# Roy-Kid/ADMP

Measured on AMD Instinct MI355X. Metric: ns/day (electrostatics get_forces per 1 fs step, polarizable PME incl. SCF, moving atoms), higher is better.
Workload: dtype f64; 1 GPU; water_pol_1024 (BASELINE configs[1]): 1024 polarizable MPID waters = 3072 atoms, seeded liquid box L=31.289 A, rc 4 A, f64; n_atoms=3072, n_pairs=42510, pair_list=fixed during the timed steps, parallelism=single GPU

## Files before the change

### admp_amd/_lib.py

```python
import ctypes

import numpy as np
import os

_HERE = os.path.dirname(os.path.abspath(__file__))
LIB_PATH = os.environ.get('ADMP_HIP_LIB') or os.path.join(_HERE, 'lib', 'libadmp_hip.so')

_c = ctypes
_vp, _i32, _i64, _dbl = _c.c_void_p, _c.c_int, _c.c_int64, _c.c_double
_u32, _u64 = _c.c_uint32, _c.c_uint64
_dp = _c.POINTER(_c.c_double)
_ip = _c.POINTER(_c.c_int)

PROTOTYPES = {
    'admp_version': (_c.c_char_p, []),
    'admp_create': (_i32, [_c.POINTER(_vp), _i32, _i32]),
    'admp_destroy': (_i32, [_vp]),
    'admp_last_error': (_c.c_char_p, [_vp]),
    'admp_set_stream': (_i32, [_vp, _vp]),
    'admp_use_default_stream': (_i32, [_vp]),
    'admp_synchronize': (_i32, [_vp]),
    'admp_set_topology': (_i32, [_vp, _i32, _vp, _vp, _vp, _vp, _vp]),
    'admp_set_ewald': (_i32, [_vp, _dbl, _i32, _i32, _i32, _i32, _i32]),
    'admp_set_pairs': (_i32, [_vp, _i64, _vp, _i32]),
    'admp_share_neighbors': (_i32, [_vp, _vp]),
    'admp_num_pairs': (_i64, [_vp]),
    'admp_set_cutoff': (_i32, [_vp, _dbl]),
    'admp_set_dipole_source': (_i32, [_vp, _vp]),
    'admp_pme_energy_grad': (_i32, [_vp, _vp, _dp, _vp, _vp, _vp, _i32, _dp, _dp, _dp, _vp, _i32, _dbl, _dp, _vp, _vp,
                                    _ip, _ip, _i32]),
    'admp_pme_energy_fixed_dipoles': (_i32, [_vp, _vp, _dp, _vp, _vp, _vp, _i32, _dp, _dp, _vp, _dp, _vp, _vp, _vp]),
    'admp_pme_box_grad': (_i32, [_vp, _vp, _dp, _vp, _vp, _vp, _i32, _dp, _dp, _vp, _dp, _dp]),
    'admp_disp_box_grad': (_i32, [_vp, _vp, _dp, _vp, _i32, _i32, _dp, _dp, _dp]),
    'admp_tt_box_grad': (_i32, [_vp, _vp, _dp, _vp, _i32, _dp, _dp, _dp]),
    'admp_local_frames': (_i32, [_vp, _vp, _dp, _vp]),
    'admp_set_option': (_i32, [_vp, _i32, _i32]),
    'admp_disp_energy_grad': (_i32, [_vp, _vp, _dp, _vp, _i32, _i32, _dp, _dp, _vp, _i32]),
    'admp_prune_pairs': (_i32, [_vp, _vp, _dp, _dbl]),
    'admp_disp_set_types': (_i32, [_vp, _i32, _vp, _dp]),
    'admp_tt_energy_grad': (_i32, [_vp, _vp, _dp, _vp, _i32, _dp, _dp, _vp, _i32]),
    'admp_pair_program_build': (_i32, [_vp, _c.c_char_p, _i32, _ip]),
    'admp_pair_program_energy_grad': (_i32, [_vp, _i32, _vp, _dp, _vp, _i32, _dp, _dp, _vp, _i32]),
    'admp_disp_param_grad': (_i32, [_vp, _vp, _dp, _vp, _i32, _i32, _dp, _vp]),
    'admp_tt_param_grad': (_i32, [_vp, _vp, _dp, _vp, _i32, _dp, _vp]),
    'admp_thole_sums': (_i32, [_vp, _vp, _dp, _vp, _vp, _vp, _i32, _dp, _dp, _vp, _vp, _vp]),
    'admp_pscale_grad': (_i32, [_vp, _vp, _dp, _vp, _vp, _vp, _i32, _dp, _dp, _vp, _dp]),
    'admp_mscale_grad': (_i32, [_vp, _i32, _vp, _dp, _vp, _i32, _i32, _dp, _i32]),
    'admp_md_bonded': (_i32, [_vp, _vp, _dp, _i32, _vp, _vp, _i32, _vp, _vp, _vp, _vp]),
    'admp_md_kick_drift': (_i32, [_vp, _i32, _vp, _vp, _vp, _vp, _dbl, _dbl, _vp]),
    'admp_md_langevin': (_i32, [_vp, _i32, _vp, _vp, _vp, _vp, _dbl, _dbl, _dbl, _dbl, _u64, _u64, _vp]),
    'admp_md_random': (_i32, [_vp, _i32, _i64, _u64, _u64, _u32, _vp]),
    'admp_md_bonded_box': (_i32, [_vp, _vp, _dp, _i32, _vp, _vp, _i32, _vp, _vp, _vp, _vp]),
    'admp_md_virial': (_i32, [_vp, _i32, _vp, _vp, _vp, _vp, _u64, _u64, _vp]),
    'admp_md_scale': (_i32, [_vp, _i32, _vp, _vp, _dbl]),
    'admp_md_mts_plan': (_i32, [_vp, _i32, _i32, _vp, _vp, _i32, _vp, _vp, _i32]),
    'admp_md_mts_step': (_i32, [_vp, _i32, _vp, _vp, _vp, _vp, _dp, _dbl, _dbl, _i32, _dbl, _dbl, _u64, _u64, _vp, _vp]),
    'admp_md_mts_info': (_i32, [_vp, _c.POINTER(_i64)]),
    'admp_md_con_plan': (_i32, [_vp, _i32, _i32, _vp, _vp, _i32]),
    'admp_md_con_step': (_i32, [_vp, _i32, _vp, _vp, _vp, _vp, _dp, _dbl, _dbl, _dbl, _dbl, _u64, _u64, _dbl, _i32, _vp]),
    'admp_md_con_kick': (_i32, [_vp, _i32, _vp, _vp, _vp, _vp, _dp, _dbl, _dbl, _dbl, _i32, _vp, _vp]),
    'admp_md_con_project': (_i32, [_vp, _i32, _vp, _vp, _vp, _dp, _dbl, _i32, _vp]),
    'admp_md_con_info': (_i32, [_vp, _c.POINTER(_i64)]),
    'admp_md_mol_plan': (_i32, [_vp, _i32, _vp, _i32]),
    'admp_md_mol_sums': (_i32, [_vp, _i32, _vp, _vp, _vp, _vp, _dp, _u64, _u64, _vp]),
    'admp_md_mol_scale': (_i32, [_vp, _i32, _vp, _vp, _vp, _dp, _dbl, _dbl]),
    'admp_md_mol_info': (_i32, [_vp, _c.POINTER(_i64)]),
    'admp_md_fire_step': (_i32, [_vp, _i32, _vp, _vp, _vp, _vp, _dp, _dbl, _u64, _vp]),
    'admp_md_vrescale': (_i32, [_vp, _i32, _vp, _vp, _vp, _dbl, _i64, _dbl, _dbl, _u64, _u64, _u64, _vp]),
    'admp_neighbor_count': (_i32, [_vp, _i32, _vp, _dp, _dbl, _c.POINTER(_i64)]),
    'admp_neighbor_fill': (_i32, [_vp, _vp]),
    'admp_set_pairs_from_positions': (_i32, [_vp, _vp, _dp, _dbl]),
    'admp_slab_configure': (_i32, [_vp, _i32, _i32]),
    'admp_slab_info': (_i32, [_vp, _c.POINTER(_i64)]),
    'admp_scf_stats': (_i32, [_vp, _c.POINTER(_i64), _i32]),
    'admp_scf_aspc': (_i32, [_vp, _i32, _i32, _dbl]),
    'admp_scf_aspc_reset': (_i32, [_vp]),
    'admp_scf_aspc_info': (_i32, [_vp, _c.POINTER(_i64), _dp]),
    'admp_xpass_stats':(_i32, [_vp, _c.POINTER(_i64), _i32]),
    'admp_plane_mfma_stats': (_i32, [_vp, _c.POINTER(_i64), _i32]),
    'admp_plane_mfma_stats4': (_i32, [_vp, _c.POINTER(_i64), _i32]),
    'admp_mesh_convolve': (_i32, [_vp, _dp, _i32, _vp, _i32, _dp, _ip]),
    'admp_slab_mesh_convolve': (_i32, [_vp, _dp, _i32, _vp, _i32, _dp, _ip]),
    'admp_slab_lists': (_i32, [_vp, _i32, _i32, _ip, _ip, _ip, _ip, _ip, _ip, _ip, _ip, _ip, _c.POINTER(_i64)]),
    'admp_pair_real': (_i32, [_vp, _vp, _dp, _vp, _vp, _vp, _i32, _dp, _dp, _vp, _vp, _i32, _i32, _i32, _dp, _vp, _vp, _vp, _ip]),
    'admp_pair_rider_stats': (_i32, [_vp, _c.POINTER(_i64), _i32]),
    'admp_mesh_spread': (_i32, [_vp, _vp, _dp, _vp, _vp, _vp, _vp, _i32, _i32, _i32, _vp, _ip]),
    'admp_mesh_gather': (_i32, [_vp, _vp, _dp, _vp, _vp, _vp, _vp, _vp, _i32, _i32, _dp, _vp, _vp, _vp, _ip]),
    'admp_set_comm': (_i32, [_vp, _vp]),
    'admp_slab_home': (_i32, [_vp, _vp, _ip, _ip]),
    'admp_rccl_unique_id': (_i32, [_vp]),
    'admp_rccl_create': (_i32, [_c.POINTER(_vp), _i32, _vp, _i32, _i32]),
    'admp_rccl_destroy': (_i32, [_vp]),
    'admp_rccl_abort': (_i32, [_vp]),
    'admp_rccl_stats': (_i32, [_vp, _c.POINTER(_i64), _c.POINTER(_i64), _i32]),
    'admp_rccl_all_reduce': (_i32, [_vp, _vp, _i64, _i32, _i32, _vp]),
    'admp_rccl_all_to_all_v': (_i32, [_vp, _vp, _c.POINTER(_i64), _vp, _c.POINTER(_i64), _i32, _vp]),
    'admp_rccl_shift': (_i32, [_vp, _vp, _vp, _i64, _i32, _i32, _vp]),
    'admp_rccl_version': (_i32, [_ip]),
    'admp_rccl_last_error': (_c.c_char_p, []),
    'admp_set_comm_rccl': (_i32, [_vp, _vp]),
    'admp_profile_enable': (_i32, [_vp, _i32]),
    'admp_profile_filter': (_i32, [_vp, _c.c_char_p]),
    'admp_profile_reset': (_i32, [_vp]),
    'admp_profile_count': (_i32, [_vp]),
    'admp_profile_entry': (_i32, [_vp, _i32, _c.POINTER(_c.c_char_p), _dp, _c.POINTER(_i64)]),
}

T_I32, T_F32, T_F64 = 0, 1, 2
OP_SUM, OP_MAX = 0, 1
TAGS = {1: 'ghost_planes', 2: 'transpose', 3: 'halo_dipoles', 4: 'halo_gradient', 5: 'scf_max', 6: 'energies',
        7: 'replicate_outputs'}
_i64p = _c.POINTER(_i64)
ALL_REDUCE_FN = _c.CFUNCTYPE(_i32, _vp, _vp, _i64, _i32, _i32, _i32)
ALL_TO_ALL_V_FN = _c.CFUNCTYPE(_i32, _vp, _vp, _i64p, _vp, _i64p, _i32, _i32)
SHIFT_FN = _c.CFUNCTYPE(_i32, _vp, _vp, _vp, _i64, _i32, _i32, _i32)


class AdmpComm(_c.Structure):
    _fields_ = [('ctx', _vp), ('all_reduce', ALL_REDUCE_FN), ('all_to_all_v', ALL_TO_ALL_V_FN), ('shift', SHIFT_FN)]


OPT_REFERENCE_KPOINTS = 1
OPT_KEEP_POL_SITES = 2
OPT_SIDE_STREAM = 3
OPT_ASPC_HOLD = 4
E_ARG, E_STATE = -1, -5
RCCL_ID_BYTES, RCCL_NTAGS = 128, 8
MESH_INFO_WORDS = 16
MESH_PATHS = ('rocfft', 'fused_x', 'direct_lines', 'direct_planes', 'two_level')

SPREAD_FORMS = ('scan', 'planes', 'bricks', 'plane_kernel')

_lib = None


class AdmpHipError(RuntimeError):
    pass


def load():
    global _lib
    if _lib is not None:
        return _lib
    if not os.path.exists(LIB_PATH):
        raise ImportError(
            'admp_amd: %s not found. Build it with `python -m admp_amd.build` (needs hipcc); '
            'there is no CPU fallback for the PME path.' % LIB_PATH)
    lib = ctypes.CDLL(LIB_PATH)
    for name, (res, args) in PROTOTYPES.items():
        fn = getattr(lib, name)
        fn.restype = res
        fn.argtypes = args
    _lib = lib
    return lib


def check(handle, rc, what):
    if rc != 0:
        msg = load().admp_last_error(handle)
        raise AdmpHipError('%s failed (code %d): %s' % (what, rc, msg.decode() if msg else ''))


def darr(values):
# ... 3 lines not shown
```

### admp_amd/csrc/atom_kernels.hip

```cpp
#include <cstdlib>

#include <cstring>

#include "launch.h"
#include "reduce.h"

namespace admp {

constexpr int kAtomBlock = 256;

template <class T>
__device__ __forceinline__ void load3(const T* a, int i, T o[3]) {
  o[0] = a[3 * i]; o[1] = a[3 * i + 1]; o[2] = a[3 * i + 2];
}

template <class T>
__device__ __forceinline__ void frame_of(const Topology& top, const T* pos, const Box<T>& box, int i, int& type,
                                         int& iz, int& ix, int& iy, FrameWork<T>& w) {
  type = top.axis_type[i];
  iz = top.axis_idx[3 * i];
  ix = top.axis_idx[3 * i + 1];
  iy = top.axis_idx[3 * i + 2];
  T p[3], pz[3] = {0, 0, 0}, px[3] = {0, 0, 0}, py[3] = {0, 0, 0};
  load3(pos, i, p);
  if (iz >= 0) load3(pos, iz, pz); else if (type != NoAxisType) type = NoAxisType;
  if (ix >= 0) load3(pos, ix, px);
  if (iy >= 0) load3(pos, iy, py);
  local_frame_fwd(type, box, p, pz, px, py, w);
}

template <class T>
__global__ __launch_bounds__(kAtomBlock) void k_prepare_sites(Topology top, const T* __restrict__ pos,
                                                              const T* __restrict__ Qlocal,
                                                              const T* __restrict__ Ucart, const T* __restrict__ pol,
                                                              const T* __restrict__ thole, Box<T> box,
                                                              Site<T>* __restrict__ sites, double* zero_next,
                                                              RecipGeom<T> g, int4* __restrict__ bases,
                                                              int* __restrict__ act_list, int* __restrict__ act_count,
                                                              const int* __restrict__ cls, int* __restrict__ cls_flags,
                                                              RQ4<T>* __restrict__ rq, T* __restrict__ Ucopy,
                                                              const int* __restrict__ list, int nlist) {
  int i = blockIdx.x * kAtomBlock + threadIdx.x;
  if (zero_next && i < E_WORDS) zero_next[i] = 0.0;
  if (list) {
    if (i >= nlist) return;
    i = list[i];
  }
  if (act_list) {
    __shared__ int wcnt[kAtomBlock / 64], wbase;
    const bool act = i < top.na && pol && pol[i] > T(0);
    const unsigned long long m = __ballot(act);
    const int lane = threadIdx.x & 63, wave = threadIdx.x >> 6;
    if (lane == 0) wcnt[wave] = __popcll(m);
    __syncthreads();
    if (threadIdx.x == 0) {
      int tot = 0;
      for (int w = 0; w < kAtomBlock / 64; ++w) { const int c = wcnt[w]; wcnt[w] = tot; tot += c; }
      wbase = tot ? atomicAdd(act_count, tot) : 0;
    }
    __syncthreads();
    if (act) act_list[wbase + wcnt[wave] + __popcll(m & ((1ull << lane) - 1ull))] = i;
  }
  if (i >= top.na) return;
  int type, iz, ix, iy;
  FrameWork<T> w;
  frame_of(top, pos, box, i, type, iz, ix, iy, w);
  T ql[9], cx[3], cy[3], cz[3];
#pragma unroll
  for (int k = 0; k < 9; ++k) ql[k] = Qlocal[9 * i + k];
  Site<T> s;
  frame_cols(w.X, w.Y, w.Z, cx, cy, cz);
  rot_harm(ql, cx, cy, cz, s.Q);
  load3(pos, i, s.r);
  if (Ucart) {
    s.U[0] = Ucart[3 * i + 2]; s.U[1] = Ucart[3 * i]; s.U[2] = Ucart[3 * i + 1];
    if (Ucopy) { Ucopy[3 * i] = s.U[1]; Ucopy[3 * i + 1] = s.U[2]; Ucopy[3 * i + 2] = s.U[0]; }
  } else {
    s.U[0] = s.U[1] = s.U[2] = T(0);
  }
  T a = pol ? pol[i] : T(0);
  s.p6 = a > T(0) ? (T)pow((double)a, 1.0 / 6.0) : T(0);
  s.thole = thole ? thole[i] : T(0);
  s.pad[0] = s.pad[1] = s.pad[2] = T(0);
  if (s.p6 == T(0) && s.U[0] == T(0) && s.U[1] == T(0) && s.U[2] == T(0)) {
    bool mono = true;
#pragma unroll
    for (int k = 1; k < 9; ++k) mono = mono && ql[k] == T(0);
    s.pad[0] = mono ? T(1) : T(0);
  }
  if (cls_flags) {
    const bool was = cls && cls[i] != 0, is = s.pad[0] == T(1) && s.p6 == T(0);
    const int f = was && !is ? CLS_STALE : (!was && is ? CLS_BETTER : 0);
    if (f && !(*(volatile int*)cls_flags & f)) atomicOr(cls_flags, f);
  }
  sites[i] = s;
  if (rq) { RQ4<T> q; q.v[0] = s.r[0]; q.v[1] = s.r[1]; q.v[2] = s.r[2]; q.v[3] = s.Q[0]; rq[i] = q; }
  if (bases) {
    int b[3];
#pragma unroll
    for (int d = 0; d < 3; ++d) grid_ref(g, s.r, d, b[d]);
    const int dims[3] = {g.nloc0, g.K[1], g.K[2]};
    bases[i] = make_int4(b[0], b[1], b[2], brick_code(b, dims, make_bricks(dims)));
  }
}

template <class T>
__global__ __launch_bounds__(kAtomBlock) void k_site_classes(int na, const Site<T>* __restrict__ sites, int* __restrict__ cls) {
  const int i = blockIdx.x * kAtomBlock + threadIdx.x;
  if (i < na) cls[i] = site_is_mono(sites[i]) ? 1 : 0;
}

template <class T>
__global__ __launch_bounds__(kAtomBlock) void k_jacobi_delta(int n_act, const int* __restrict__ act,
                                                             const T* __restrict__ pol, const T* __restrict__ field,
                                                             T* __restrict__ Ucart, Site<T>* __restrict__ sites,
                                                             Site<T>* __restrict__ isites,
                                                             const unsigned long long* __restrict__ gate,
                                                             unsigned long long gate_bits, T relax) {
  const int slot = blockIdx.x * kAtomBlock + threadIdx.x;
  if (slot >= n_act) return;
  const int i = act[slot];
  const bool on = !gate || *gate >= gate_bits;
  const T s = on ? -pol[i] * T(1.0 / kDielectric) * relax : T(0);
  const T dx = field[3 * i] * s, dy = field[3 * i + 1] * s, dz = field[3 * i + 2] * s;
  Ucart[3 * i] += dx; Ucart[3 * i + 1] += dy; Ucart[3 * i + 2] += dz;
  Site<T> r = sites[i];
  r.U[0] += dz; r.U[1] += dx; r.U[2] += dy;
  r.pad[0] = dz; r.pad[1] = dx; r.pad[2] = dy;
  sites[i] = r;
#pragma unroll
  for (int k = 0; k < 9; ++k) r.Q[k] = T(0);
  r.U[0] = dz; r.U[1] = dx; r.U[2] = dy;
  isites[slot] = r;
}

template <class T>
__global__ __launch_bounds__(kAtomBlock) void k_aspc_predict(long n, AspcSets<T> h, T* __restrict__ out) {
  const long i = (long)blockIdx.x * kAtomBlock + threadIdx.x;
  if (i >= n) return;
  double acc = 0.0;
#pragma unroll
  for (int j = 0; j < kAspcMaxSets; ++j)
    if (j < h.n) acc += h.B[j] * (double)h.U[j][i];
  out[i] = (T)acc;
}

template <class T>
__global__ __launch_bounds__(kAtomBlock) void k_local_frames(Topology top, const T* __restrict__ pos, Box<T> box,
                                                             T* __restrict__ out) {
  int i = blockIdx.x * kAtomBlock + threadIdx.x;
  if (i >= top.na) return;
  int type, iz, ix, iy;
  FrameWork<T> w;
  frame_of(top, pos, box, i, type, iz, ix, iy, w);
#pragma unroll
  for (int k = 0; k < 3; ++k) { out[9 * i + k] = w.X[k]; out[9 * i + 3 + k] = w.Y[k]; out[9 * i + 6 + k] = w.Z[k]; }
}
template <class T>
void launch_local_frames(hipStream_t st, const Topology& top, const T* pos, const Box<T>& box, T* out) {
  k_local_frames<T><<<(top.na + kAtomBlock - 1) / kAtomBlock, kAtomBlock, 0, st>>>(top, pos, box, out);
}
template void launch_local_frames<float>(hipStream_t, const Topology&, const float*, const Box<float>&, float*);
template void launch_local_frames<double>(hipStream_t, const Topology&, const double*, const Box<double>&, double*);

template <class T>
__global__ __launch_bounds__(kAtomBlock) void k_field_finish(int na, const Site<T>* __restrict__ sites,
                                                             const T* __restrict__ pol, const T* __restrict__ Ucart,
                                                             const T* __restrict__ fld_pair,
                                                             const T* __restrict__ fld_recip, T kappa,
                                                             T* __restrict__ field, unsigned long long* fmax_bits,
                                                             const int* __restrict__ list, const int* __restrict__ n_dev) {
  const int slot = blockIdx.x * kAtomBlock + threadIdx.x;
  if (n_dev) na = min(na, *n_dev);
  double fm = 0.0;
  if (slot < na) {
    const int i = list ? list[slot] : slot;
    const T a = pol[i];
    T fx, fy, fz;
    total_field(sites[i], a, Ucart + 3 * i, fld_pair + 3 * i, fld_recip + 3 * i, kappa, fx, fy, fz);
    field[3 * i] = fx; field[3 * i + 1] = fy; field[3 * i + 2] = fz;
    if (a > T(0.001)) fm = fmax(fabs((double)fx), fmax(fabs((double)fy), fabs((double)fz)));
  }
  fm = block_reduce_max<kAtomBlock>(fm);
  if (threadIdx.x == 0 && fm > 0.0) atomicMax(fmax_bits, nonneg_bits(fm));
}

template <class T>
__global__ __launch_bounds__(kAtomBlock) void k_finish(Topology top, const T* __restrict__ pos, Box<T> box,
                                                       const Site<T>* __restrict__ sites, const T* __restrict__ pol,
                                                       const T* __restrict__ Ucart, int lpol, T kappa,
                                                       T* __restrict__ pot, T* __restrict__ grad,
                                                       T* __restrict__ dQlocal, double* energies,
                                                       const int* __restrict__ list, int nlist) {
  const int slot = blockIdx.x * kAtomBlock + threadIdx.x;
  double eself = 0.0, epen = 0.0;
  if (slot < nlist) {
    const int i = list ? list[slot] : slot;
    T f[3];
    self_factors(kappa, f);
    const Site<T>& s = sites[i];
    T Qt[9], P[9];
#pragma unroll
    for (int k = 0; k < 9; ++k) { Qt[k] = s.Q[k]; P[k] = pot[9 * i + k]; }
    if (lpol) { Qt[1] += s.U[0]; Qt[2] += s.U[1]; Qt[3] += s.U[2]; }
// ... 371 lines not shown
    FrameWork<T> w;
    frame_of(top, pos, box, i, type, iz, ix, iy, w);
    if (type != NoAxisType) {
      T f[3], P[9], tau[3], gp[3], gz[3], gx[3], gy[3], p[3];
      self_factors(kappa, f);
      total_potential(sites[i], pot + 9 * (size_t)i, lpol, f, P, nullptr);
      multipole_torque(P, sites[i].Q, tau);
      local_frame_bwd(type, w, tau, gp, gz, gx, gy);
      load3(pos, i, p);
      const int member[3] = {iz, type != Zonly ? ix : -1, (type == ZBisect || type == ThreeFold) ? iy : -1};
      const T* gk[3] = {gz, gx, gy};
      for (int m = 0; m < 3; ++m) {
        if (member[m] < 0) continue;
        T q[3], sh[3];
        load3(pos, member[m], q);
        const T d[3] = {q[0] - p[0], q[1] - p[1], q[2] - p[2]};
        if (!image_shift(box, d, sh)) continue;
        for (int a = 0; a < 3; ++a)
          for (int b = 0; b < 3; ++b) acc[3 * a + b] += (double)sh[a] * (double)gk[m][b];
      }
    }
  }
#pragma unroll
  for (int k = 0; k < 9; ++k) {
    const double v = block_reduce_sum<kAtomBlock>(acc[k]);
    if (threadIdx.x == 0 && v != 0.0) atomicAdd(&vir[k], v);
  }
}

template <class T>
__global__ __launch_bounds__(kAtomBlock) void k_scalar_sites(int na, const T* __restrict__ pos, const T* __restrict__ vals,
                                                             int stride, int chan, SelfCoefs self_coefs,
                                                             Site<T>* __restrict__ sites, double* energies, RecipGeom<T> g,
                                                             int4* __restrict__ bases) {
  chan += blockIdx.y;
  sites += (size_t)blockIdx.y * na;
  const double self_coef = self_coefs.c[blockIdx.y];
  const int i = blockIdx.x * kAtomBlock + threadIdx.x;
  double s2 = 0.0;
  if (i < na) {
    Site<T> s;
    load3(pos, i, s.r);
    const T c = vals[(long)stride * i + chan];
    s.Q[0] = c;
#pragma unroll
    for (int k = 1; k < 9; ++k) s.Q[k] = T(0);
    s.U[0] = s.U[1] = s.U[2] = T(0);
    s.p6 = s.thole = T(0);
    s.pad[0] = s.pad[1] = s.pad[2] = T(0);
    sites[i] = s;
    s2 = (double)c * (double)c;
    if (bases && blockIdx.y == 0) {
      int b[3];
#pragma unroll
      for (int d = 0; d < 3; ++d) grid_ref(g, s.r, d, b[d]);
      const int dims[3] = {g.nloc0, g.K[1], g.K[2]};
      bases[i] = make_int4(b[0], b[1], b[2], brick_code(b, dims, make_bricks(dims)));
    }
  }
  s2 = block_reduce_sum<kAtomBlock>(s2);
  if (threadIdx.x == 0) atomicAdd(&energies[E_SELF], self_coef * s2);
}

template <class T>
__global__ __launch_bounds__(kAtomBlock) void k_scale_add(int na, const T* __restrict__ vals, int stride, int chan,
                                                          const T* __restrict__ v, T* __restrict__ grad, int nch) {
  const int i = blockIdx.x * kAtomBlock + threadIdx.x;
  if (i >= na) return;
  T gx = 0, gy = 0, gz = 0;
  for (int b = 0; b < nch; ++b) {
    const T c = vals[(long)stride * i + chan + b];
    const T* vb = v + (size_t)b * 3 * na;
    gx += c * vb[3 * i]; gy += c * vb[3 * i + 1]; gz += c * vb[3 * i + 2];
  }
  grad[3 * i] += gx; grad[3 * i + 1] += gy; grad[3 * i + 2] += gz;
}

static inline int nblk(int n) { return (n + kAtomBlock - 1) / kAtomBlock; }

template <class T>
void launch_prepare_sites(hipStream_t st, const Topology& top, const T* pos, const T* Qlocal, const T* Ucart,
                          const T* pol, const T* thole, const Box<T>& box, Site<T>* sites, double* zero_next,
                          const RecipGeom<T>& g, int4* bases, int* act_list, int* act_count, const int* cls,
                          int* cls_flags, RQ4<T>* rq, T* Ucopy, const int* list, int nlist) {
  const int n = list ? nlist : top.na;
  if (n <= 0 && !zero_next) return;
  k_prepare_sites<T><<<nblk(n > E_WORDS || !zero_next ? (n > 0 ? n : 1) : E_WORDS), kAtomBlock, 0, st>>>(
      top, pos, Qlocal, Ucart, pol, thole, box, sites, zero_next, g, bases, list ? nullptr : act_list,
      list ? nullptr : act_count, cls, cls_flags, rq, Ucopy, list, nlist);
}
template <class T>
void launch_site_classes(hipStream_t st, int na, const Site<T>* sites, int* cls) {
  if (na > 0) k_site_classes<T><<<nblk(na), kAtomBlock, 0, st>>>(na, sites, cls);
}
template <class T>
void launch_field_finish(hipStream_t st, int na, const Site<T>* sites, const T* pol, const T* Ucart, const T* fld_pair,
                         const T* fld_recip, T kappa, T* field, unsigned long long* fmax_bits, const int* list,
                         const int* n_dev) {
  k_field_finish<T><<<nblk(na), kAtomBlock, 0, st>>>(na, sites, pol, Ucart, fld_pair, fld_recip, kappa, field, fmax_bits, list,
                                                     n_dev);
}
template <class T>
void launch_jacobi_delta(hipStream_t st, int n_act, const int* act, const T* pol, const T* field, T* Ucart, Site<T>* sites,
                         Site<T>* isites, const unsigned long long* gate, double gate_min, double relax) {
  unsigned long long bits;
  std::memcpy(&bits, &gate_min, sizeof(bits));
  if (n_act > 0)
    k_jacobi_delta<T><<<nblk(n_act), kAtomBlock, 0, st>>>(n_act, act, pol, field, Ucart, sites, isites, gate, bits, (T)relax);
}
template <class T>
void launch_aspc_predict(hipStream_t st, long n, const AspcSets<T>& h, T* out) {
  if (n > 0) k_aspc_predict<T><<<(unsigned)((n + kAtomBlock - 1) / kAtomBlock), kAtomBlock, 0, st>>>(n, h, out);
}
template <class T>
void launch_finish(hipStream_t st, const Topology& top, const T* pos, const Box<T>& box, const Site<T>* sites,
                   const T* pol, const T* Ucart, int lpol, T kappa, T* pot, T* grad, T* dQlocal, double* energies,
                   const int* list, int nlist, const FieldFin<T>& ff, const int* slab_bits) {
  const int gmin = env_int("ADMP_FINISH_GROUPS_MIN", 8192);
  if ((!list || slab_bits) && top.ngroups > 0 && top.na > gmin) {
    if (top.rows_blk && env_flag("ADMP_FINISH_ROWS", true))
      k_finish_rows<T><<<top.nrowblk < 1024 ? top.nrowblk : 1024, kFinishBlock, 0, st>>>(top, box, sites, pol, lpol, kappa, pot, grad,
                                                                                         dQlocal, energies, ff,
                                                                                         list ? slab_bits : nullptr);
    else
      k_finish_groups<T><<<nblk(top.ngroups), kAtomBlock, 0, st>>>(top, pos, box, sites, pol, Ucart, lpol, kappa, pot, grad,
                                                                   dQlocal, energies, ff, list ? slab_bits : nullptr);
    return;
  }
  if (!list && top.inv_ptr)
  {
    static const int lanes4_max = env_int("ADMP_FINISH4_MAX", 8192);
    if (top.na <= lanes4_max)
      k_finish_pull<T, 4><<<nblk(4 * top.na), kAtomBlock, 0, st>>>(top, pos, box, sites, pol, Ucart, lpol, kappa, pot, grad,
                                                                   dQlocal, energies, ff);
    else
      k_finish_pull<T, 1><<<nblk(top.na), kAtomBlock, 0, st>>>(top, pos, box, sites, pol, Ucart, lpol, kappa, pot, grad,
                                                               dQlocal, energies, ff);
  }
  else
    k_finish<T><<<nblk(nlist), kAtomBlock, 0, st>>>(top, pos, box, sites, pol, Ucart, lpol, kappa, pot, grad, dQlocal,
                                                    energies, list, nlist);
}

template <class T>
void launch_frame_virial(hipStream_t st, const Topology& top, const T* pos, const Box<T>& box, const Site<T>* sites,
                         int lpol, T kappa, const T* pot, double* vir, const int* list, int nlist) {
  const int n = list ? nlist : top.na;
  if (n > 0) k_frame_virial<T><<<nblk(n), kAtomBlock, 0, st>>>(top, pos, box, sites, lpol, kappa, pot, vir, list, nlist);
}
template void launch_frame_virial<float>(hipStream_t, const Topology&, const float*, const Box<float>&, const Site<float>*,
                                         int, float, const float*, double*, const int*, int);
template void launch_frame_virial<double>(hipStream_t, const Topology&, const double*, const Box<double>&,
                                          const Site<double>*, int, double, const double*, double*, const int*, int);

template <class T>
void launch_scalar_sites(hipStream_t st, int na, const T* pos, const T* vals, int stride, int chan, double self_coef,
                         Site<T>* sites, double* energies) {
  SelfCoefs sc;
  sc.c[0] = self_coef;
  k_scalar_sites<T><<<nblk(na), kAtomBlock, 0, st>>>(na, pos, vals, stride, chan, sc, sites, energies, RecipGeom<T>(), nullptr);
}
template <class T>
void launch_scalar_sites_batch(hipStream_t st, int na, const T* pos, const T* vals, int stride, int nch,
                               const double* self_coefs, Site<T>* sites, double* energies, const RecipGeom<T>* g, int4* bases) {
  SelfCoefs sc;
  for (int b = 0; b < nch && b < 3; ++b) sc.c[b] = self_coefs[b];
  k_scalar_sites<T><<<dim3(nblk(na), nch), kAtomBlock, 0, st>>>(na, pos, vals, stride, 0, sc, sites, energies,
                                                                 g ? *g : RecipGeom<T>(), g ? bases : nullptr);
}
template <class T>
void launch_scale_add(hipStream_t st, int na, const T* vals, int stride, int chan, const T* v, T* grad, int nch) {
  k_scale_add<T><<<nblk(na), kAtomBlock, 0, st>>>(na, vals, stride, chan, v, grad, nch);
}

#define INST(T)                                                                                                        \
  template void launch_scalar_sites<T>(hipStream_t, int, const T*, const T*, int, int, double, Site<T>*, double*);      \
  template void launch_scale_add<T>(hipStream_t, int, const T*, int, int, const T*, T*, int);                           \
  template void launch_scalar_sites_batch<T>(hipStream_t, int, const T*, const T*, int, int, const double*, Site<T>*,   \
                                             double*, const RecipGeom<T>*, int4*);                                      \
  template void launch_prepare_sites<T>(hipStream_t, const Topology&, const T*, const T*, const T*, const T*, const T*, \
                                        const Box<T>&, Site<T>*, double*, const RecipGeom<T>&, int4*, int*, int*,       \
                                        const int*, int*, RQ4<T>*, T*, const int*, int);                                \
  template void launch_site_classes<T>(hipStream_t, int, const Site<T>*, int*);                                         \
  template void launch_field_finish<T>(hipStream_t, int, const Site<T>*, const T*, const T*, const T*, const T*, T, T*,  \
                                       unsigned long long*, const int*, const int*);                                    \
  template void launch_jacobi_delta<T>(hipStream_t, int, const int*, const T*, const T*, T*, Site<T>*, Site<T>*,        \
                                       const unsigned long long*, double, double);                                    \
  template void launch_aspc_predict<T>(hipStream_t, long, const AspcSets<T>&, T*);                                      \
  template void launch_finish<T>(hipStream_t, const Topology&, const T*, const Box<T>&, const Site<T>*, const T*,        \
                                 const T*, int, T, T*, T*, T*, double*, const int*, int, const FieldFin<T>&, const int*);
INST(float)
INST(double)
#undef INST

}
```

### admp_amd/csrc/dft_kernels.hip

```cpp
#include "dft_lines.h"
#include "env.h"
#include "mfma.h"
#include "plane_mfma_plan.h"

namespace admp {

int dft_tile_cols(int N) { return dft_cols(N, dft_kq(), 0, 0); }
template <class T, int KQ, int JS>
__global__ __launch_bounds__(kDftBlock) void k_dft_z_r2c(int N, int nlines, int NL, int TK, const T* __restrict__ mesh,
                                                        Cx<T>* __restrict__ spec, const Cx<T>* __restrict__ twg,
                                                        long mesh_stride, long spec_stride) {
  mesh += blockIdx.y * mesh_stride;
  spec += blockIdx.y * spec_stride;
  const int H = (N - 1) / 2, Kh = N / 2 + 1;
  Cx<T>* tw = reinterpret_cast<Cx<T>*>(dft_smem);
  Cx<T>* p = tw + N;
  T* x0 = reinterpret_cast<T*>(p + H * NL);
  T* xn = x0 + NL;
  const int line0 = blockIdx.x * NL;
  const int nl = min(NL, nlines - line0);
  for (int t = threadIdx.x; t < N; t += kDftBlock) tw[t] = twg[t];
  for (int t = threadIdx.x; t < H * nl; t += kDftBlock) {
    const int l = t / H, jj = t - l * H;
    const T* x = mesh + (long)(line0 + l) * N;
// ... 225 lines not shown
  __syncthreads();
  double e = 0.0;
  auto combine = [&](Cx<T>* s, const T* G) {
    Cx<T> y[NTP];
#pragma unroll
    for (int ty = 0; ty < NTP; ++ty) y[ty] = Cx<T>{T(0), T(0)};
    double en = 0.0;
#pragma unroll
    for (int ch = 0; ch < 3; ++ch) {
      if (ch >= mix.nch) break;
      Cx<T> Sp{T(0), T(0)};
#pragma unroll
      for (int ty = 0; ty < NTP; ++ty) { const T cc = (T)mix.c[ch][ty]; Sp.re += cc * s[ty].re; Sp.im += cc * s[ty].im; }
      en += (double)G[ch] * ((double)Sp.re * Sp.re + (double)Sp.im * Sp.im);
#pragma unroll
      for (int ty = 0; ty < NTP; ++ty) { const T cg = (T)mix.c[ch][ty] * G[ch]; y[ty].re += cg * Sp.re; y[ty].im += cg * Sp.im; }
    }
#pragma unroll
    for (int ty = 0; ty < NTP; ++ty) s[ty] = y[ty];
    return en;
  };
#pragma unroll
  for (int u = 0; u < KQ; ++u) {
    const int t = threadIdx.x + u * kDftBlock;
    if (t >= H * NCt) continue;
    const int jj = t / NCt, cc = t - jj * NCt;
    Cx<T> s1[NTP], s2[NTP];
#pragma unroll
    for (int ty = 0; ty < NTP; ++ty) s1[ty] = s2[ty] = Cx<T>{T(0), T(0)};
    if (cc < ncp) {
      const int k1 = 1 + jj, k2 = N - 1 - jj, kz = col0 + cc;
#pragma unroll
      for (int ty = 0; ty < NTP; ++ty) { s1[ty] = S[k1 * NC + ty * NCt + cc]; s2[ty] = S[k2 * NC + ty * NCt + cc]; }
      const double w = (kz == 0 || ((K3 & 1) == 0 && kz == K3 / 2)) ? 0.5 : 1.0;
      const T G1[3] = {Gp[u][0][0], Gp[u][1][0], Gp[u][2][0]}, G2[3] = {Gp[u][0][1], Gp[u][1][1], Gp[u][2][1]};
      e += w * (combine(s1, G1) + combine(s2, G2));
    }
#pragma unroll
    for (int ty = 0; ty < NTP; ++ty)
      ab[jj * NC + ty * NCt + cc] = PairCx<T>{s1[ty].re + s2[ty].re, s1[ty].im + s2[ty].im, s1[ty].re - s2[ty].re, s1[ty].im - s2[ty].im};
  }
  if ((int)threadIdx.x < NCt) {
    const int cc = threadIdx.x;
    Cx<T> a[NTP], b[NTP];
#pragma unroll
    for (int ty = 0; ty < NTP; ++ty) a[ty] = b[ty] = Cx<T>{T(0), T(0)};
    if (cc < ncp) {
      const int kz = col0 + cc;
      const double w = (kz == 0 || ((K3 & 1) == 0 && kz == K3 / 2)) ? 0.5 : 1.0;
#pragma unroll
      for (int ty = 0; ty < NTP; ++ty) a[ty] = S[ty * NCt + cc];
      e += w * combine(a, G0);
      if ((N & 1) == 0) {
#pragma unroll
        for (int ty = 0; ty < NTP; ++ty) b[ty] = S[(N / 2) * NC + ty * NCt + cc];
        e += w * combine(b, Gn);
      }
    }
#pragma unroll
    for (int ty = 0; ty < NTP; ++ty) { x0[ty * NCt + cc] = a[ty]; xn[ty * NCt + cc] = b[ty]; }
  }
  __syncthreads();
  if (task) {
    Cx<T> Xk[KQ], Xnk[KQ];
    dft_pair_outputs_js<T, +1, KQ, JS>(N, k, NC, ab + c, x0[c], xn[c], tw, half, Xk, Xnk);
    Cx<T>* sp = spec + (long)cty * spec_tstride + base + ccol;
#pragma unroll
    for (int q = 0; q < KQ; ++q) {
      const int kq = g + q * TK;
      if (kq < Kh) {
        if (JS == 1 || half == 0) sp[(long)kq * jstride] = Xk[q];
        if ((JS == 1 || half == 1) && kq != 0 && 2 * kq != N) sp[(long)(N - kq) * jstride] = Xnk[q];
      }
    }
  }
  e = block_reduce_sum<kDftBlock>(e);
  if (threadIdx.x == 0) atomicAdd(&energies[slot], e);
}

constexpr int kZyBlock = 1024;

#ifdef ADMP_ZY_TRACE
__device__ long long* g_zy_trace;
#define ZY_TRACE(slot) do { if (threadIdx.x == 0) g_zy_trace[((blockIdx.z * gridDim.y + blockIdx.y) * gridDim.x + blockIdx.x) * 8 + (slot)] = wall_clock64(); } while (0)
#define ZY_TRACE_END(slot) do { __syncthreads(); ZY_TRACE(slot); } while (0)
#else
#define ZY_TRACE(slot) do {} while (0)
#define ZY_TRACE_END(slot) do {} while (0)
#endif

template <class T>
struct ZyLayout {
  size_t tw3, tw2, a, x0, b, total;
  __host__ __device__ ZyLayout(int N2, int N3) {
    const size_t H3 = (size_t)(N3 - 1) / 2, Kh = (size_t)N3 / 2 + 1;
    tw3 = 0;
    tw2 = tw3 + sizeof(Cx<T>) * N3;
    a = tw2 + sizeof(Cx<T>) * N2;
    const size_t fa = sizeof(Cx<T>) * H3 * N2, ia = sizeof(Cx<T>) * N2 * Kh;
    x0 = a + (fa > ia ? fa : ia);
    b = x0 + sizeof(Cx<T>) * N2;
    total = b + sizeof(Cx<T>) * N2 * Kh;
  }
};

constexpr int kZyW = 42;
constexpr int kZyScan = 3;
constexpr int kZySpreadMaxAtoms = 8192;
template <class T>
__host__ __device__ inline int zy_spread_sub(int N2, int N3) {
  const int Kh = N3 / 2 + 1;
  const long spare = (long)sizeof(Cx<T>) * N2 * Kh - (long)sizeof(unsigned short) * kZyScan * kZyBlock;
  const long n = spare / (long)(kZyW * sizeof(T) + 2 * sizeof(int));
  return n > kZyBlock / 3 ? kZyBlock / 3 : (int)n;
}
template <class T>
__device__ __forceinline__ void zy_plane_spread(const PlaneSpread<T>& sp, int px, int N2, int N3, Cx<T>* p, T* x0, T* xn,
                                                unsigned char* scratch, int SUB) {
  __shared__ int s_nhit;
  unsigned short* hits = reinterpret_cast<unsigned short*>(scratch);
  T* wts = reinterpret_cast<T*>(hits + kZyScan * kZyBlock);
  int* ebase = reinterpret_cast<int*>(wts + (size_t)SUB * kZyW);
  const int H3 = (N3 - 1) / 2;
  const Site<T>* sites = sp.sites + (size_t)blockIdx.y * sp.na;
  for (int t = threadIdx.x; t < H3 * N2; t += kZyBlock) p[t] = Cx<T>{T(0), T(0)};
  for (int t = threadIdx.x; t < 2 * N2; t += kZyBlock) x0[t] = T(0);
  const RecipGeom<T>& g = sp.g;
  for (int c0 = 0; c0 < sp.na; c0 += kZyScan * kZyBlock) {
    if (threadIdx.x == 0) s_nhit = 0;
    __syncthreads();
    int bx[kZyScan];
#pragma unroll
    for (int r = 0; r < kZyScan; ++r) {
      const int i = c0 + (int)threadIdx.x + r * kZyBlock;
      bx[r] = -1000;
      if (i < sp.na) {
        if (sp.bases) bx[r] = sp.bases[i].x;
        else {
          const T rr[3] = {sites[i].r[0], sites[i].r[1], sites[i].r[2]};
          (void)grid_ref(g, rr, 0, bx[r]);
        }
      }
    }
#pragma unroll
    for (int r = 0; r < kZyScan; ++r) {
      int a = px - bx[r];
      if (a < 0) a += g.K[0];
      if (bx[r] >= 0 && a < 6)
        hits[atomicAdd(&s_nhit, 1)] = (unsigned short)((c0 + (int)threadIdx.x + r * kZyBlock) | (a << 13));
    }
    __syncthreads();
    const int nhit = s_nhit;
    const int nsub = (nhit + SUB - 1) / SUB, per = nsub > 0 ? (nhit + nsub - 1) / nsub : 0;
    for (int sub = 0; sub < nhit; sub += per) {
      const int cnt = min(per, nhit - sub);
      if ((int)threadIdx.x < 3 * cnt) {
        const int e = threadIdx.x / 3, part = threadIdx.x - 3 * e;
        const int h = hits[sub + e];
        const Site<T>& site = sites[h & 0x1fff];
        T* w = wts + e * kZyW;
        const T r[3] = {site.r[0], site.r[1], site.r[2]};
        int base;
        T M[6], D1[6], D2[6], D3[6];
        const T f = grid_ref(g, r, part, base);
        bspline6(f, M, D1, D2, D3);
        if (part == 0) {
          const int a = h >> 13;
          T m0 = T(0), d0 = T(0), e0 = T(0);
#pragma unroll
          for (int k = 0; k < 6; ++k)
            if (k == a) { m0 = M[k]; d0 = D1[k]; e0 = D2[k]; }
          T Q[9], c1[3], c2[6];
#pragma unroll
          for (int k = 0; k < 9; ++k) Q[k] = site.Q[k];
          if (sp.lpol) { Q[1] += site.U[0]; Q[2] += site.U[1]; Q[3] += site.U[2]; }
          fold_multipole(g, Q, c1, c2);
          w[0] = Q[0] * m0 + c1[0] * d0 + c2[0] * e0;
          w[1] = c1[1] * m0 + c2[3] * d0;
          w[2] = c2[1] * m0;
          w[3] = c1[2] * m0 + c2[4] * d0;
          w[4] = c2[5] * m0;
          w[5] = c2[2] * m0;
        } else {
          const int o = part == 1 ? 6 : 24;
#pragma unroll
          for (int k = 0; k < 6; ++k) { w[o + k] = M[k]; w[o + 6 + k] = D1[k]; w[o + 12 + k] = D2[k]; }
          ebase[2 * e + part - 1] = base;
        }
      }
      __syncthreads();
      for (int task = threadIdx.x; task < cnt * 6; task += kZyBlock) {
        const int e = task / 6, b = task - e * 6;
        const T* w = wts + e * kZyW;
        const T m1 = w[6 + b], d1 = w[12 + b], e1 = w[18 + b];
        const T P0 = w[0] * m1 + w[1] * d1 + w[2] * e1;
        const T P1 = w[3] * m1 + w[4] * d1;
        const T P2 = w[5] * m1;
        const int jb = wrap_add(ebase[2 * e], b, N2), bz = ebase[2 * e + 1];
#pragma unroll
        for (int c = 0; c < 6; ++c) {
          const T v = P0 * w[24 + c] + P1 * w[30 + c] + P2 * w[36 + c];
          const int jc = wrap_add(bz, c, N3);
          T* dst;
          if (jc == 0) dst = &x0[jb];
          else if (jc <= H3) dst = &p[(jc - 1) * N2 + jb].re;
          else if (2 * jc == N3) dst = &xn[jb];
          else dst = &p[(N3 - 1 - jc) * N2 + jb].im;
          atomicAdd(dst, v);
        }
      }
      __syncthreads();
    }
  }
  for (int t = threadIdx.x; t < H3 * N2; t += kZyBlock) {
    const Cx<T> ab = p[t];
    p[t] = Cx<T>{ab.re + ab.im, ab.re - ab.im};
  }
}

template <class T, int SIGN>
__device__ __forceinline__ void dft_y_unit_rows(int N, int H, int KP, int ncols, int ib, int kl, int ct, bool w0, bool wn,
                                                const Cx<T>* Z, const Cx<T>* tw, Cx<T>* out, int os) {
  typedef typename Mfma<T>::Acc Acc;
  const int lane = threadIdx.x & 63, hi = plane_mfma_pos0(lane);
  const int i = ib + (lane & 15), c = plane_mfma_col(ct, lane), comp = plane_mfma_comp(lane);
  TwIdx ti(i < kl ? i : 0, hi, N);
  const bool live = c < ncols;
  const T* zc = reinterpret_cast<const T*>(Z + (live ? c : 0)) + comp;
  const int rs = 2 * ncols;
  struct Ops { Cx<T> w; T b[2]; };
  auto fetch = [&](Ops& o, int kk) {
    o.w = tw[ti.m];
    ti.step();
    const bool ok = live && kk < H;
    o.b[0] = ok ? zc[(1 + kk) * rs] : T(0);
    o.b[1] = ok ? zc[(N - 1 - kk) * rs] : T(0);
  };
  Acc P = {0, 0, 0, 0}, R = {0, 0, 0, 0};
  T s0 = T(0);
  auto mul = [&](const Ops& o) {
    s0 += o.b[0];
    P = Mfma<T>::mma(o.w.re, o.b[0], P);
    R = Mfma<T>::mma(o.w.im, o.b[1], R);
  };
  Ops A, B;
  fetch(A, hi);
  for (int kk = hi; kk < KP; kk += 8) {
    const bool two = kk + 4 < KP;
    if (two) fetch(B, kk + 4);
    mul(A);
    if (kk + 8 < KP) fetch(A, kk + 8);
    if (two) mul(B);
  }
  const T x0 = zc[0], xn = (N & 1) ? T(0) : zc[(N / 2) * rs];
  T* o = reinterpret_cast<T*>(out + (live ? c : 0)) + comp;
#pragma unroll
  for (int r = 0; r < 4; ++r) {
    const int k = 1 + ib + (lane >> 4) + 4 * r;
    const T other = __shfl_xor(R[r], 8, 64);
    if (live && k <= kl) {
      T base = x0 + P[r];
      if ((N & 1) == 0) base += (k & 1) ? -xn : xn;
      const T q = comp ? T(SIGN) * other : -T(SIGN) * other;
      o[2 * (long)k * os] = base + q;
      o[2 * (long)(N - k) * os] = base - q;
    }
  }
  if (w0 || wn) {
    T s1 = (hi & 1) ? s0 : -s0;
    s0 += __shfl_xor(s0, 16, 64); s1 += __shfl_xor(s1, 16, 64);
    s0 += __shfl_xor(s0, 32, 64); s1 += __shfl_xor(s1, 32, 64);
    if (hi == 0 && live) {
      if (w0) o[0] = x0 + s0 + xn;
      if (wn && (N & 1) == 0) o[2 * (long)(N / 2) * os] = x0 + s1 + (((N / 2) & 1) ? -xn : xn);
    }
  }
}

template <class T, int SIGN>
__device__ __forceinline__ void dft_y_unit(const PlaneMfmaPlan& mp, int u, const Cx<T>* Z, const Cx<T>* tw, Cx<T>* out, int os) {
  const int mt = u % mp.MT, ct = u / mp.MT;
  dft_y_unit_rows<T, SIGN>(mp.N, mp.H, mp.KP, mp.ncols, plane_mfma_tw_row(mt, 0), mp.H, ct, mt == 0, mt == 0, Z, tw, out, os);
}
template <class T>
__device__ __forceinline__ void dft_y_unit_inv(const PlaneMfmaInvYPlan& yp, int u, const Cx<T>* Z, const Cx<T>* tw, Cx<T>* V) {
  const int mt = u % yp.MT, ct = u / yp.MT;
  dft_y_unit_rows<T, +1>(yp.N, yp.H, yp.KP, yp.ncols, plane_mfma_inv_y_kb(yp, mt) - 1, plane_mfma_inv_y_ke(yp, mt) - 1, ct,
                         mt == 0 && yp.s.own0, mt == 0 && yp.s.ownn, Z, tw, V, yp.ncols);
}

template <class T>
__device__ __forceinline__ void dft_z_unit(const PlaneMfmaZPlan& zp, int u, const Cx<T>* p, const T* x0, const T* xn,
                                           const Cx<T>* tw, Cx<T>* Z) {
  typedef typename Mfma<T>::Acc Acc;
  const int N = zp.N, H = zp.H, mt = u % zp.MT, lt = u / zp.MT;
  const int lane = threadIdx.x & 63, hi = lane >> 4;
  const int kt = plane_mfma_z_tw_k(zp, mt, lane), l = plane_mfma_z_line(lt, lane);
  TwIdx ti((kt <= N / 2 ? kt : 0) - 1, hi, N);
  const bool live = l < zp.nlines;
  const Cx<T>* pl = p + (live ? l : 0);
  struct Ops { Cx<T> w, v; };
  auto fetch = [&](Ops& o, int kk) {
    o.w = tw[ti.m];
    ti.step();
    o.v = (live && kk < H) ? pl[kk * zp.nlines] : Cx<T>{T(0), T(0)};
  };
  Acc P = {0, 0, 0, 0}, R = {0, 0, 0, 0};
  auto mul = [&](const Ops& o) {
    P = Mfma<T>::mma(o.w.re, o.v.re, P);
    R = Mfma<T>::mma(o.w.im, o.v.im, R);
  };
  Ops A, B;
  fetch(A, hi);
  for (int kk = hi; kk < zp.KP; kk += 8) {
    const bool two = kk + 4 < zp.KP;
    if (two) fetch(B, kk + 4);
    mul(A);
    if (kk + 8 < zp.KP) fetch(A, kk + 8);
    if (two) mul(B);
  }
  if (live) {
    const T a0 = x0[l], an = xn[l];
#pragma unroll
    for (int r = 0; r < 4; ++r) {
      const int k = plane_mfma_z_out_k(zp, mt, lane, r);
      if (k < zp.k0 + zp.nout) {
        T re = a0 + P[r];
        if ((N & 1) == 0) re += (k & 1) ? -an : an;
        Z[l * zp.nout + k - zp.k0] = Cx<T>{re, -R[r]};
      }
    }
  }
}

template <class T, int KQ, bool SPREAD, bool MF = false>
__global__ __launch_bounds__(kZyBlock) void k_dft_zy_fwd(int N2, int N3, const T* __restrict__ mesh, Cx<T>* __restrict__ spec,
                                                         const Cx<T>* __restrict__ tw2g, const Cx<T>* __restrict__ tw3g,
                                                         long mesh_stride, long spec_stride, PlaneSpread<T> sp) {
  const ZyLayout<T> L(N2, N3);
  const int H3 = (N3 - 1) / 2, Kh = N3 / 2 + 1, H2 = (N2 - 1) / 2;
  const int kz0 = (int)(((long)Kh * blockIdx.z) / gridDim.z), kz1 = (int)(((long)Kh * (blockIdx.z + 1)) / gridDim.z);
  const int Kl = kz1 - kz0;
  Cx<T>* tw3 = reinterpret_cast<Cx<T>*>(dft_smem + L.tw3);
  Cx<T>* tw2 = reinterpret_cast<Cx<T>*>(dft_smem + L.tw2);
  Cx<T>* p = reinterpret_cast<Cx<T>*>(dft_smem + L.a);
  T* x0 = reinterpret_cast<T*>(dft_smem + L.x0);
  T* xn = x0 + N2;
  Cx<T>* Z = reinterpret_cast<Cx<T>*>(dft_smem + L.b);
  const T* plane = mesh + blockIdx.y * mesh_stride + (long)blockIdx.x * N2 * N3;
  Cx<T>* out = spec + blockIdx.y * spec_stride + (long)blockIdx.x * N2 * Kh;
  ZY_TRACE(0);
  for (int t = threadIdx.x; t < N3; t += kZyBlock) tw3[t] = tw3g[t];
  for (int t = threadIdx.x; t < N2; t += kZyBlock) tw2[t] = tw2g[t];
  if (SPREAD) {
    zy_plane_spread<T>(sp, (int)blockIdx.x, N2, N3, p, x0, xn, dft_smem + L.b, zy_spread_sub<T>(N2, N3));
  } else {
    for (int t = threadIdx.x; t < H3 * N2; t += kZyBlock) {
      const int l = t / H3, jj = t - l * H3;
      const T* x = plane + (long)l * N3;
      const T a = x[1 + jj], b = x[N3 - 1 - jj];
      p[jj * N2 + l] = Cx<T>{a + b, a - b};
    }
    for (int l = threadIdx.x; l < N2; l += kZyBlock) {
      x0[l] = plane[(long)l * N3];
      xn[l] = (N3 & 1) ? T(0) : plane[(long)l * N3 + N3 / 2];
    }
  }
  __syncthreads();
  ZY_TRACE(1);
  const int TK3 = (Kl + KQ - 1) / KQ;
  const PlaneMfmaZPlan zp = plane_mfma_z_plan(N3, kz0, Kl, N2, kZyBlock / 64);
  const bool zshare = MF && zp.nunits > 0;
  if (zshare) {
    for (int u = threadIdx.x >> 6; u < zp.nunits; u += zp.Wm) dft_z_unit<T>(zp, u, p, x0, xn, tw3, Z);
  }
  for (int task = zshare ? N2 * TK3 : (int)threadIdx.x; task < N2 * TK3; task += kZyBlock) {
    const int l = task / TK3, g = task - l * TK3;
    int k[KQ];
#pragma unroll
    for (int q = 0; q < KQ; ++q) k[q] = (g + q * TK3 < Kl) ? kz0 + g + q * TK3 : 0;
    Cx<T> X[KQ];
    rdft_outputs<T, KQ>(N3, k, N2, p + l, x0[l], xn[l], tw3, X);
#pragma unroll
    for (int q = 0; q < KQ; ++q)
      if (g + q * TK3 < Kl) Z[l * Kl + g + q * TK3] = X[q];
  }
  __syncthreads();
  ZY_TRACE(2);
  for (int t = threadIdx.x; t < H2 * Kl; t += kZyBlock) {
    const int jj = t / Kl, c = t - jj * Kl;
    const Cx<T> a = Z[(1 + jj) * Kl + c], b = Z[(N2 - 1 - jj) * Kl + c];
    Z[(1 + jj) * Kl + c] = Cx<T>{a.re + b.re, a.im + b.im};
    Z[(N2 - 1 - jj) * Kl + c] = Cx<T>{a.re - b.re, a.im - b.im};
  }
  __syncthreads();
  ZY_TRACE(3);
  const int Kh2 = N2 / 2 + 1, TK2 = (Kh2 + KQ - 1) / KQ;
  if (MF) {
    const PlaneMfmaPlan mp = plane_mfma_y_plan(N2, Kl, kZyBlock / 64);
    const int wave = threadIdx.x >> 6, nv = Kl - mp.nm;
    if (wave < mp.Wm) {
      for (int u = wave; u < mp.nunits; u += mp.Wm) dft_y_unit<T, -1>(mp, u, Z, tw2, out + kz0, Kh);
    } else {
      for (int task = (int)threadIdx.x - 64 * mp.Wm; task < TK2 * nv; task += kZyBlock - 64 * mp.Wm) {
        const int g = task / nv, c = mp.nm + task - g * nv;
        int k[KQ];
#pragma unroll
        for (int q = 0; q < KQ; ++q) k[q] = (g + q * TK2 < Kh2) ? g + q * TK2 : 0;
        Cx<T> Xk[KQ], Xnk[KQ];
        dft_pair_outputs_rows<T, -1, KQ>(N2, k, Kl, Z + c, tw2, Xk, Xnk);
#pragma unroll
        for (int q = 0; q < KQ; ++q) {
          const int kq = g + q * TK2;
          if (kq < Kh2) {
            out[(long)kq * Kh + kz0 + c] = Xk[q];
            if (kq != 0 && 2 * kq != N2) out[(long)(N2 - kq) * Kh + kz0 + c] = Xnk[q];
          }
        }
      }
    }
    ZY_TRACE_END(4);
    return;
  }
  for (int task = threadIdx.x; task < TK2 * Kl; task += kZyBlock) {
    const int g = task / Kl, c = task - g * Kl;
    int k[KQ];
#pragma unroll
    for (int q = 0; q < KQ; ++q) k[q] = (g + q * TK2 < Kh2) ? g + q * TK2 : 0;
    Cx<T> Xk[KQ], Xnk[KQ];
    dft_pair_outputs_rows<T, -1, KQ>(N2, k, Kl, Z + c, tw2, Xk, Xnk);
#pragma unroll
    for (int q = 0; q < KQ; ++q) {
      const int kq = g + q * TK2;
      if (kq < Kh2) {
        out[(long)kq * Kh + kz0 + c] = Xk[q];
        if (kq != 0 && 2 * kq != N2) out[(long)(N2 - kq) * Kh + kz0 + c] = Xnk[q];
      }
    }
// ... 329 lines not shown
```

### admp_amd/csrc/engine.hip

```cpp
#include <hip/hip_runtime.h>
#include <hip/hiprtc.h>
#include <rocfft/rocfft.h>

#include <algorithm>
#include <array>
#include <cmath>
#include <cstdio>
#include <cstring>
#include <map>
#include <memory>
#include <mutex>
#include <set>
#include <string>
#include <functional>
#include <vector>

#include "../../include/admp_hip.h"
#include "dev_buf.h"
#include "dft_math.h"
#include "disp_plan.h"
#include "handle.h"
#include "launch.h"
#include "rccl_comm.h"
#include "scf_policy.h"
#include "scf_aspc.h"

using namespace admp;

namespace {

#define FFT_TRY(x)                                                                                       \
  do {                                                                                                   \
    rocfft_status s_ = (x);                                                                              \
    if (s_ != rocfft_status_success) throw Err{ADMP_E_FFT, std::string(#x) + ": rocfft status " + std::to_string((int)s_)}; \
  } while (0)

std::once_flag g_fft_once;

struct EngineBase : HandleCtx {
  virtual ~EngineBase() {}
  Topology top;
  NbrTable nbr;
  bool have_top = false, have_ewald = false, have_pairs = false;
  double kappa = 0;
  int K[3] = {0, 0, 0};
  int lmax = 2, lpol = 0;
  admp_comm comm{};
  bool have_comm = false;
  admp_rccl* rccl = nullptr;
  void comm_fail(const char* what, int rc) {
    if (rccl) throw Err{ADMP_E_COMM, std::string(what) + ": " + rccl_error()};
    throw Err{ADMP_E_COMM, std::string("communicator callback ") + what + " returned " + std::to_string(rc)};
  }
  void c_all_reduce(void* buf, int64_t n, int dtype, int op, int tag) {
    const int rc = rccl ? rccl_all_reduce(rccl, stream, buf, n, dtype, op, tag) : comm.all_reduce(comm.ctx, buf, n, dtype, op, tag);
    if (rc != 0) comm_fail("all_reduce", rc);
  }
  void c_all_to_all_v(const void* send, const int64_t* sc, void* recv, const int64_t* rc_, int dtype, int tag) {
    const int rc = rccl ? rccl_all_to_all_v(rccl, stream, send, sc, recv, rc_, dtype, tag)
                        : comm.all_to_all_v(comm.ctx, send, sc, recv, rc_, dtype, tag);
    if (rc != 0) comm_fail("all_to_all_v", rc);
  }
  void c_shift(const void* send, void* recv, int64_t n, int dtype, int to_next, int tag) {
    const int rc = rccl ? rccl_shift(rccl, stream, send, recv, n, dtype, to_next, tag)
                        : comm.shift(comm.ctx, send, recv, n, dtype, to_next, tag);
    if (rc != 0) comm_fail("shift", rc);
  }
  int64_t scf_stats[8] = {0, 0, 0, 0, 0, 0, 0, 0};
  int64_t xpass_stats[2] = {0, 0};
  int64_t plane_mfma_stats[2] = {0, 0};
  int64_t plane_mfma_stats4[4] = {0, 0, 0, 0};
  int64_t pair_rider_stats[2] = {0, 0};
  AspcRing aspc;
  int64_t aspc_calls[3] = {0, 0, 0};
  double aspc_resid = 0.0;
  int aspc_hold = 0;
  bool aspc_dirty = false;
  void aspc_off() { aspc.configure(-1, 1, 0.0); aspc_dirty = false; }
  const void* U_src = nullptr;
  const void* U_src_now = nullptr;
  double cutoff = 0.0;
  int ref_korder = 0;
  int keep_pol_sites = 0;
  int side_stream_on = 1;
  virtual void after_error() {}
  long nbr_gen = 0;
  NbrTable nbr_full;
  bool pruned = false;
  void unprune() {
    if (!pruned) return;
    nbr = nbr_full;
    nbr_full = NbrTable();
    pruned = false;
    ++nbr_gen;
  }
  EngineBase* nbr_src = nullptr;
  long nbr_src_gen = -1;
  static std::set<EngineBase*>& live() { static std::set<EngineBase*> s; return s; }
  static std::mutex& live_mu() { static std::mutex m; return m; }
  static bool is_live(EngineBase* e) { std::lock_guard<std::mutex> g(live_mu()); return live().count(e) != 0; }
  void detach_shared() {
    if (!nbr_src) return;
    nbr = NbrTable();
    nbr_src = nullptr; nbr_src_gen = -1;
    have_pairs = false;
    ++nbr_gen;
  }
  void adopt_shared() {
    if (!nbr_src) return;
    if (!is_live(nbr_src)) { nbr = NbrTable(); nbr_src = nullptr; have_pairs = false; throw Err{ADMP_E_ARG, "the handle the neighbour table was borrowed from has been destroyed"}; }
    if (!nbr_src->have_pairs || nbr_src->top.na != top.na) { nbr = NbrTable(); have_pairs = false; return; }
    if (nbr_src_gen != nbr_src->nbr_gen || nbr.col != nbr_src->nbr.col || nbr.order != nbr_src->nbr.order ||
        nbr.order_plain != nbr_src->nbr.order_plain) {
      if (nbr_src->stream != stream) HIP_TRY(hipStreamSynchronize(nbr_src->stream));
      nbr = nbr_src->nbr;
      nbr_src_gen = nbr_src->nbr_gen;
      ++nbr_gen;
    }
    have_pairs = true;
  }
  void share_neighbors(EngineBase* src) {
    ARG_CHECK(have_top, "admp_set_topology must precede admp_share_neighbors");
    if (!src) { detach_shared(); return; }
    ARG_CHECK(src != this && !src->nbr_src, "the lender must own its neighbour table");
    ARG_CHECK(src->have_top && src->top.na == top.na && src->device == device, "handles of different systems / devices");
    unprune();
    if (!nbr_src) nbr.free_all();
    nbr = NbrTable();
    nbr_src = src; nbr_src_gen = -1;
    have_pairs = false;
    adopt_shared();
  }
  DevBuf scan_scratch;
  size_t scan_bytes = 0;

  virtual void set_ewald(double kappa_, int K1, int K2, int K3, int lmax_, int lpol_) = 0;
  virtual void pme(const void* pos, const double* box, const void* Ql, const void* pol, const void* thole, int ns,
                   const double* mS, const double* pS, void* U, int max_cycle, double thresh, double* E, void* dpos,
                   void* dQl, int* ncyc, int* conv, int on_device) = 0;
  virtual void pme_at_U(const void* pos, const double* box, const void* Ql, const void* pol, const void* thole, int ns,
                        const double* mS, const double* pS, const void* U, double* E, void* dpos, void* dU, void* dQl) = 0;
  virtual void local_frames(const void* pos, const double* box, void* out) = 0;
  virtual void mesh_convolve(const double* box, int which, void* data, int on_device, double* E_out, int32_t* info) = 0;
  virtual void slab_mesh_convolve(const double* box, int which, void* data, int on_device, double* E_out, int32_t* info) = 0;
  virtual void pair_program_eval(int id, const void* pos, const double* box, const void* par, int ns, const double* mS,
                                 double* E, void* dpos, int on_device) = 0;

  struct PairProgram { hipModule_t mod = nullptr; hipFunction_t fn = nullptr; int n_params = 0; };
  std::vector<PairProgram> programs;
  int pair_program_build(const char* source, int n_params) {
    ARG_CHECK(source && n_params >= 0 && n_params <= 16, "bad pair program");
    hiprtcProgram prog = nullptr;
    auto rtc = [&](hiprtcResult r, const char* what) {
      if (r != HIPRTC_SUCCESS) throw Err{ADMP_E_HIP, std::string(what) + ": " + hiprtcGetErrorString(r)};
// ... 218 lines not shown
  }

  void set_pairs(int64_t n_rows, const int32_t* pairs, int on_device) {
    unprune();
    ARG_CHECK(have_top, "admp_set_topology must precede admp_set_pairs");
    ARG_CHECK(n_rows >= 0, "negative pair count");
    detach_shared();
    DevBuf staged;
    const int* dev = pairs;
    if (!on_device && n_rows > 0) {
      staged.need(sizeof(int) * 2 * (size_t)n_rows);
      HIP_TRY(hipMemcpyAsync(staged.p, pairs, sizeof(int) * 2 * (size_t)n_rows, hipMemcpyHostToDevice, stream));
      dev = staged.as<int>();
    }
    {
      TIMED("nbr_build");
      if (nbr.built) { (void)hipFree(nbr.built); nbr.built = nullptr; }
      int rc = build_neighbour_table(stream, top, n_rows, dev, nbr, &scan_scratch.p, &scan_bytes);
      if (rc != 0) throw Err{ADMP_E_HIP, std::string("build_neighbour_table: ") + hipGetErrorString((hipError_t)rc)};
      apply_classes();
      order_rows();
    }
    HIP_TRY(hipStreamSynchronize(stream));
    have_pairs = true;
    ++nbr_gen;
  }
};

struct SlabState {
  DevBuf owner, owner_prev, mig, bits, counts, totals, lists, imp, exp, mig_in, mig_out, sendb, recvb, ghost, pack, tbuf;
  int prev_na = -1;
  int64_t min_cnt[kSlabMaxRanks], mout_cnt[kSlabMaxRanks];
  int n_min = 0, n_mout = 0;
  int64_t tr_send[kSlabMaxRanks], tr_recv[kSlabMaxRanks];
  int64_t imp_cnt[kSlabMaxRanks], exp_cnt[kSlabMaxRanks];
  int n_home = 0, n_act = 0, n_imp = 0, n_exp = 0;
  bool tracked = false;
  const int* home = nullptr;
  const int* rows = nullptr;
  const int* act = nullptr;
};

template <class T>
struct Engine : EngineBase {
  DevBuf sites, grad, pot, fld_pair, fld_recip, field, energies_d;
  bool fmax_clean = false, slot_clean[E_SLOTS] = {false};
  int ehalf = 0;
  bool other_clean = false;
  void* energies_seen = nullptr;
  double* Eh = nullptr;
  double* Ed_cur() { return energies_d.as<double>() + (size_t)ehalf * E_WORDS; }
  DevBuf s_pos, s_Q, s_pol, s_thole, s_U, s_out, s_dQ, s_par;
  DevBuf mesh, spec, gtabs[4], fft_work, binv_d, bin_cells, bin_sorted, bin_scan, bin_cells_ind, bin_sorted_ind;
  T* gtab_cur = nullptr;
  BinScratch bins, bins_ind;
  rocfft_plan plan_f = nullptr, plan_b = nullptr, plan_xf = nullptr, plan_xb = nullptr;
  rocfft_plan plan2_f = nullptr, plan2_b = nullptr;
  int fx_khp = 0;
  bool use_fx = false;
  DevBuf fx_tw;
  rocfft_execution_info info_f = nullptr;
  int planK[3] = {0, 0, 0}, planR = 0, planRank = 0;
  DevBuf home_list;
  DevBuf act_tmp;
  DevBuf onehot_d, tcount_d;
  void* onehot_for = nullptr;
  DevBuf act_d, isites, mesh2;
  IndTable ind;
  DevBuf cut_end, cut_col, cut_iend, cut_icol;
  NbrTable cut_nbr;
  IndTable cut_ind;
  bool cut_on = false;
  const NbrTable& wnbr() const { return cut_on ? cut_nbr : nbr; }
  const IndTable& wind() const { return cut_on ? cut_ind : ind; }
  long act_gen = 0, act_top_na = -1;
  int act_n = -1;
  bool act_fresh = false;
  long ind_nbr_gen = -1, ind_act_gen = -1;
  long eval_seq = 0, ind_bins_eval = -1, ind_bins_gen = -1;
  int ind_bins_n = -1;
  const int* ind_bins_at = nullptr;
  DevBuf dft_tw;
  DevBuf bases_d;
  bool use_dft = false;
  bool use_pfa = false;
  PfaPlan pfa;
  DevBuf pfa_tw, pfa_fmap, pfa_ptab, gtab_nat;
  struct TabKey { double box[9] = {0}, kappa = -1; int K[3] = {0, 0, 0}, Y0 = 0, ref = 0; bool pfa = false; } tabkey[4];
  DevBuf xctab, xctab_flag;
  bool xctab_ok = false;
  static bool xcirc_on() { static const bool on = env_flag("ADMP_DFT_XCIRC", true); return on; }
  static int tab_slot(int which) { return which == 1 ? 0 : (which == 6 ? 1 : (which == 8 ? 2 : 3)); }
  static_assert(kScfChainSteps == E_CHAIN, "one residual word per chained Jacobi step");
  ScfHistory scf;
  bool mono_ok = false;

  ~Engine() override {
    destroy_plans();
    free_topology();
    if (ind.end) (void)hipFree(ind.end);
    if (ind.col) (void)hipFree(ind.col);
    cells.release();
    free_programs();
    if (Eh) (void)hipHostFree(Eh);
    prof.destroy();
    if (side) { (void)hipStreamSynchronize(side); (void)hipStreamDestroy(side); }
    if (ev_fork) (void)hipEventDestroy(ev_fork);
    if (ev_join) (void)hipEventDestroy(ev_join);
    if (own_stream && stream) (void)hipStreamDestroy(stream);
  }

  void destroy_plans() {
    if (plan_f) rocfft_plan_destroy(plan_f);
    if (plan_b) rocfft_plan_destroy(plan_b);
    if (plan_xf) rocfft_plan_destroy(plan_xf);
    if (plan_xb) rocfft_plan_destroy(plan_xb);
    if (plan2_f) rocfft_plan_destroy(plan2_f);
    if (plan2_b) rocfft_plan_destroy(plan2_b);
    for (int k = 0; k < 4; ++k) {
      if (plan2n_f[k]) rocfft_plan_destroy(plan2n_f[k]);
      if (plan2n_b[k]) rocfft_plan_destroy(plan2n_b[k]);
      plan2n_f[k] = plan2n_b[k] = nullptr;
    }
    if (info_f) rocfft_execution_info_destroy(info_f);
    plan_f = plan_b = plan_xf = plan_xb = plan2_f = plan2_b = nullptr;
    use_fx = false;
    info_f = nullptr;
    planK[0] = planK[1] = planK[2] = 0;
  }

  void set_ewald(double kappa_, int K1, int K2, int K3, int lmax_, int lpol_) override {
    ARG_CHECK(kappa_ > 0, "kappa must be positive");
    ARG_CHECK(K1 >= 2 && K2 >= 2 && K3 >= 2, "PME mesh must be at least 2 points per dimension");
    ARG_CHECK(lmax_ >= 0 && lmax_ <= 2, "l > 2 (beyond quadrupole) not supported");
    kappa = kappa_; K[0] = K1; K[1] = K2; K[2] = K3; lmax = lmax_; lpol = lpol_ ? 1 : 0;
    have_ewald = true;
    aspc.drop();
    if (!lpol) aspc_off();
  }

  static constexpr int kGhost = 5;
  int X0 = 0, X1 = 0, Y0 = 0, Y1 = 0;
  void update_slab() {
    X0 = (int)((long)srank * K[0] / snranks); X1 = (int)((long)(srank + 1) * K[0] / snranks);
    Y0 = (int)((long)srank * K[1] / snranks); Y1 = (int)((long)(srank + 1) * K[1] / snranks);
    if (snranks > 1) {
      ARG_CHECK(have_comm, "slab-decomposed handle without a communicator (admp_set_comm)");
      const int64_t nh = K[2] / 2 + 1;
      for (int s = 0; s < snranks; ++s) {
        int w = (int)((long)(s + 1) * K[0] / snranks) - (int)((long)s * K[0] / snranks);
        ARG_CHECK(w >= 6, "slab decomposition needs at least 6 mesh planes per rank along x");
        int wy = (int)((long)(s + 1) * K[1] / snranks) - (int)((long)s * K[1] / snranks);
        ARG_CHECK(wy >= 1, "slab decomposition needs at least 1 mesh row per rank along y");
        sl.tr_send[s] = (int64_t)(X1 - X0) * wy * nh * 2;
        sl.tr_recv[s] = (int64_t)w * (Y1 - Y0) * nh * 2;
      }
    }
  }
  SlabState sl;
  static constexpr int real_dtype() { return sizeof(T) == 4 ? ADMP_T_F32 : ADMP_T_F64; }
  void decompose() { decompose(K[0], X0, X1, nbr.order, lpol != 0); }
  void decompose(int K0v, int X0v, int X1v, const int* order, bool with_dipoles = false) {
    const int na = top.na, N = snranks, me = srank;
    ARG_CHECK(N <= kSlabMaxRanks, "at most 28 slab ranks");
    sl.owner.need(sizeof(int) * (size_t)na);
    sl.bits.need(sizeof(int) * (size_t)na);
// ... 234 lines not shown
                                   pr, 1, len1, batch, desc));
        FFT_TRY(rocfft_plan_description_destroy(desc));
      }
      FFT_TRY(rocfft_plan_get_work_buffer_size(plan_xf, &w)); if (w > wmax) wmax = w;
      FFT_TRY(rocfft_plan_get_work_buffer_size(plan_xb, &w)); if (w > wmax) wmax = w;
      if (!fx_off && fftx_usable(K[0])) upload_fx_twiddles();
    }
    FFT_TRY(rocfft_plan_get_work_buffer_size(plan_f, &w)); if (w > wmax) wmax = w;
    FFT_TRY(rocfft_plan_get_work_buffer_size(plan_b, &w)); if (w > wmax) wmax = w;
    fft_work.need(wmax + 16);
    FFT_TRY(rocfft_execution_info_create(&info_f));
    if (wmax) FFT_TRY(rocfft_execution_info_set_work_buffer(info_f, fft_work.p, wmax));
    planK[0] = K[0]; planK[1] = K[1]; planK[2] = K[2]; planR = snranks; planRank = srank;
    for (auto& k : tabkey) k.kappa = -1;
    setup_dft();
  }

  void setup_dft() {
    use_dft = use_pfa = false;
    if (snranks != 1) return;
    const int mode = env_int("ADMP_DFT", -1);
    if (mode == 0) return;
    bool small = true, hard = false;
    for (int d = 0; d < 3; ++d) {
      small = small && K[d] >= 2 && K[d] <= 160;
      hard = hard || largest_prime_factor(K[d]) > 13;
    }
    if (mode == 2 && setup_pfa()) return;
    if (!small && hard && setup_pfa()) return;
    if (!small || !(hard || mode == 1 || mode == 2)) return;
    std::vector<T> tw(2 * (size_t)(K[0] + K[1] + K[2]));
    size_t o = 0;
    for (int d = 0; d < 3; ++d)
      for (int m = 0; m < K[d]; ++m) {
        const double th = 2.0 * M_PI * (double)m / (double)K[d];
        tw[o++] = (T)std::cos(th);
        tw[o++] = (T)std::sin(th);
      }
    dft_tw.need(tw.size() * sizeof(T));
    HIP_TRY(hipMemcpy(dft_tw.p, tw.data(), tw.size() * sizeof(T), hipMemcpyHostToDevice));
    use_dft = true;
  }
  bool setup_pfa() {
    static const bool off = !env_flag("ADMP_PFA", true);
    if (off) return false;
    for (int d = 0; d < 3; ++d)
      if (!pfa_split(K[d], &pfa.ax[d])) return false;
    pfa.Khp = pfa.ax[2].N1 * (pfa.ax[2].N2 / 2 + 1);
    std::vector<T> tw;
    for (int d = 0; d < 3; ++d) {
      pfa.tw_off[d] = (int)(tw.size() / 2);
      for (int n : {pfa.ax[d].N2, pfa.ax[d].N1})
        for (int m = 0; m < n; ++m) {
          const double th = 2.0 * M_PI * (double)m / (double)n;
          tw.push_back((T)std::cos(th));
          tw.push_back((T)std::sin(th));
        }
    }
    pfa_tw.need(tw.size() * sizeof(T));
    HIP_TRY(hipMemcpy(pfa_tw.p, tw.data(), tw.size() * sizeof(T), hipMemcpyHostToDevice));
    std::vector<int> fm((size_t)K[0] + K[1] + pfa.Khp);
    pfa_freq_of_slot(pfa.ax[0], fm.data());
    pfa_freq_of_slot(pfa.ax[1], fm.data() + K[0]);
    pfa_freq_of_zcolumn(pfa.ax[2], fm.data() + K[0] + K[1]);
    pfa_fmap.need(fm.size() * sizeof(int));
    HIP_TRY(hipMemcpy(pfa_fmap.p, fm.data(), fm.size() * sizeof(int), hipMemcpyHostToDevice));
    std::vector<int> pt((size_t)K[0] + K[1] + K[2]);
    pfa_index_table(pfa.ax[0], pt.data());
    pfa_index_table(pfa.ax[1], pt.data() + K[0]);
    pfa_index_table(pfa.ax[2], pt.data() + K[0] + K[1]);
    pfa_ptab.need(pt.size() * sizeof(int));
    HIP_TRY(hipMemcpy(pfa_ptab.p, pt.data(), pt.size() * sizeof(int), hipMemcpyHostToDevice));
    pfa.ptab[0] = pfa_ptab.as<int>(); pfa.ptab[1] = pfa.ptab[0] + K[0]; pfa.ptab[2] = pfa.ptab[1] + K[1];
    spec.need((size_t)K[0] * K[1] * pfa.Khp * 2 * sizeof(T));
    use_pfa = true;
    return true;
  }
  bool spread_fused(int n) const {
    return use_dft && !use_pfa && snranks == 1 && !ev.home && dft_zy_spread_fits<T>(K, n);
  }
  PlaneSpread<T> plane_spread(int n, const Site<T>* rows, int lp, const int4* bases) const {
    PlaneSpread<T> sp;
    sp.na = n; sp.lpol = lp; sp.sites = rows; sp.bases = bases; sp.g = ev.g;
    return sp;
  }
  bool rider_ok() const {
    static const bool on = env_flag("ADMP_FIELD_RIDER", true);
    return on && use_dft && !use_pfa && snranks == 1 && !overlap_ok();
  }
  bool pair_rider_ok() const {
    return lpol && side_stream_on && rider_ok() && env_flag("ADMP_PAIR_RIDER", true);
  }
  template <class XPass>
  void slab_convolve(T* mesh_p, T* spec_p, T* mesh_o, XPass&& xpass) {
    const size_t plane = (size_t)K[1] * K[2];
    const int nx = nxown(), ny = nyown(), nh = K[2] / 2 + 1;
    sl.ghost.need(kGhost * plane * sizeof(T));
    sl.pack.need((size_t)nx * K[1] * nh * 2 * sizeof(T));
    sl.tbuf.need((size_t)K[0] * ny * nh * 2 * sizeof(T));
    { TIMED("comm_ghost"); c_shift(mesh_p + (size_t)nx * plane, sl.ghost.p, (int64_t)(kGhost * plane), real_dtype(), 1, ADMP_TAG_GHOST); }
    { TIMED("mesh_add"); launch_mesh_add<T>(stream, (long)(kGhost * plane), mesh_p, sl.ghost.as<T>()); }
    fft_forward(mesh_p, spec_p);
    { TIMED("transpose_pack"); launch_transpose_pack<T>(stream, nx, K[1], nh, fx_khp, snranks, 0, spec_p, sl.pack.as<T>()); }
    { TIMED("comm_transpose"); c_all_to_all_v(sl.pack.p, sl.tr_send, sl.tbuf.p, sl.tr_recv, real_dtype(), ADMP_TAG_TRANSPOSE); }
    xpass(sl.tbuf.as<T>(), ny, nh);
    { TIMED("comm_transpose"); c_all_to_all_v(sl.tbuf.p, sl.tr_recv, sl.pack.p, sl.tr_send, real_dtype(), ADMP_TAG_TRANSPOSE); }
    { TIMED("transpose_pack"); launch_transpose_pack<T>(stream, nx, K[1], nh, fx_khp, snranks, 1, spec_p, sl.pack.as<T>()); }
    fft_inverse(spec_p, mesh_o);
    { TIMED("comm_ghost"); c_shift(mesh_o, mesh_o + (size_t)nx * plane, (int64_t)(kGhost * plane), real_dtype(), 0, ADMP_TAG_GHOST); }
  }
  bool convolve(T* mesh_p, T* spec_p, const T* gtab, int slot, T* accum = nullptr, T* out = nullptr,
                const PlaneSpread<T>* sp = nullptr, const PairFieldArgs<T>* rider = nullptr, const PairFullArgs<T>* prider = nullptr) {
    double* Ed = Ed_cur();
    T* mesh_o = out ? out : mesh_p;
    ARG_CHECK(!sp || (use_dft && !use_pfa && snranks == 1), "internal: plane spread on a transform path without it");
    ARG_CHECK(!(rider && rider->kind) || (use_dft && !use_pfa && snranks == 1), "internal: field rider on a transform path without it");
    ARG_CHECK(!(prider && prider->on) || (use_dft && !use_pfa && snranks == 1 && !(rider && rider->kind == 1)),
              "internal: pair rider on a transform path without it");
    if (snranks > 1) {
      slab_convolve(mesh_p, spec_p, mesh_o, [&](T* tbuf, int ny, int nh) {
        if (use_fx) {
          TIMED("fftx_kspace");
          launch_fftx_conv<T>(stream, K, fx_tw.as<T>(), tbuf, gtab, Ed, slot, nh, ny);
        } else {
          fft_x(tbuf, 0);
          { TIMED("kspace"); launch_kspace<T>(stream, K, ny, gtab, tbuf, Ed, slot); }
          fft_x(tbuf, 1);
        }
      });
      (void)accum;
      return false;
    }
    if (use_pfa) {
      const T* tw = pfa_tw.as<T>();
      { TIMED("dft_z_r2c"); launch_pfa_z<T>(stream, pfa, tw, mesh_p, spec_p, 0); }
      { TIMED("dft_y_fwd"); launch_pfa_y<T>(stream, pfa, tw, spec_p, 0); }
      DftTabs<T> tabs;
      tabs.p[0] = gtab;
      { TIMED("dft_x_kspace"); launch_pfa_x_conv<T>(stream, pfa, tw, spec_p, tabs, Ed, slot); }
      { TIMED("dft_y_inv"); launch_pfa_y<T>(stream, pfa, tw, spec_p, 1); }
      { TIMED("dft_z_c2r"); launch_pfa_z<T>(stream, pfa, tw, mesh_p, spec_p, 1); }
      return false;
    }
    if (use_dft) {
      const T* tw = dft_tw.as<T>();
      const bool planes = dft_zy_fits<T>(K);
      ARG_CHECK(!sp || planes, "internal: plane spread without the plane kernels");
      int mf = 0;
      if (planes && sp) { TIMED("dft_spread_zy_fwd"); launch_dft_zy<T>(stream, K, tw, mesh_p, spec_p, 0, 1, 0, 0, nullptr, sp, &mf); }
      else if (planes) { TIMED("dft_zy_fwd"); launch_dft_zy<T>(stream, K, tw, mesh_p, spec_p, 0, 1, 0, 0, nullptr, nullptr, &mf); }
      if (planes) { ++plane_mfma_stats[mf ? 0 : 1]; ++plane_mfma_stats4[mf ? 0 : 1]; }
      else {
        { TIMED("dft_z_r2c"); launch_dft_z<T>(stream, K, tw, mesh_p, spec_p, 0); }
        { TIMED("dft_y_fwd"); launch_dft_y<T>(stream, K, tw, spec_p, 0); }
      }
      DftTabs<T> tabs;
      tabs.p[0] = gtab;
      const T* ct = xctab_ok && gtab == gtabs[0].template as<T>() ? xctab.template as<T>() : nullptr;
      ++xpass_stats[ct ? 0 : 1];
      { TIMED("dft_x_kspace"); launch_dft_x_pass<T>(stream, K, tw, spec_p, tabs, Ed, slot, ct, rider, prider); }
      bool added;
      if (planes) {
        TIMED("dft_yz_inv");
        added = launch_dft_zy<T>(stream, K, tw, mesh_p, spec_p, 1, 1, 0, 0, accum, nullptr, &mf);
        ++plane_mfma_stats[1];
        ++plane_mfma_stats4[mf ? 2 : 3];
      }
      else {
        { TIMED("dft_y_inv"); launch_dft_y<T>(stream, K, tw, spec_p, 1); }
        { TIMED("dft_z_c2r"); added = launch_dft_z<T>(stream, K, tw, mesh_p, spec_p, 1, 1, 0, 0, accum); }
      }
      return added;
    }
    if (use_fx) {
      run_plan("rocfft_r2c_yz", plan2_f, mesh_p, spec_p);
      { TIMED("fftx_kspace"); launch_fftx_conv<T>(stream, K, fx_tw.as<T>(), spec_p, gtab, Ed, slot, fx_khp); }
      run_plan("rocfft_c2r_yz", plan2_b, spec_p, mesh_o);
      return false;
    }
    fft_forward(mesh_p, spec_p);
    { TIMED("kspace"); launch_kspace<T>(stream, K, nyown(), gtab, spec_p, Ed, slot); }
    fft_inverse(spec_p, mesh_o);
    return false;
  }

  rocfft_plan plan2n_f[4] = {nullptr, nullptr, nullptr, nullptr}, plan2n_b[4] = {nullptr, nullptr, nullptr, nullptr};
  void ensure_batched_plans(int nb) {
    ARG_CHECK(nb >= 2 && nb <= 3 && use_fx && snranks == 1, "internal: batched y-z plans");
    if (plan2n_f[nb]) return;
    make_yz_plans((size_t)nb * K[0], &plan2n_f[nb], &plan2n_b[nb]);
    size_t w = 0, wmax = 0;
    FFT_TRY(rocfft_plan_get_work_buffer_size(plan2n_f[nb], &w)); if (w > wmax) wmax = w;
    FFT_TRY(rocfft_plan_get_work_buffer_size(plan2n_b[nb], &w)); if (w > wmax) wmax = w;
    if (wmax + 16 > fft_work.bytes) {
      HIP_TRY(hipStreamSynchronize(stream));
      fft_work.need(wmax + 16);
    }
    if (fft_work.bytes > 16) FFT_TRY(rocfft_execution_info_set_work_buffer(info_f, fft_work.p, fft_work.bytes - 16));
  }
  void convolve_batch(T* mesh_p, T* spec_p, const DftTabs<T>& tabs, int nb, size_t nreal, size_t nspec, int slot) {
    ensure_batched_plans(nb);
    run_plan("rocfft_r2c_yz", plan2n_f[nb], mesh_p, spec_p);
    { TIMED("fftx_kspace");
      launch_fftx_conv_batch<T>(stream, K, fx_tw.as<T>(), spec_p, tabs, nb, (long)nspec, Ed_cur(), slot, fx_khp); }
    run_plan("rocfft_c2r_yz", plan2n_b[nb], spec_p, mesh_p);
    (void)nreal;
  }
  void convolve_dft_batch(T* mesh_p, T* spec_p, const DftTabs<T>& tabs, int nb, size_t nreal, size_t nspec, int slot,
                          const MixTab* mix = nullptr) {
    double* Ed = Ed_cur();
    if (use_pfa) {
      const T* tw = pfa_tw.as<T>();
      { TIMED("dft_z_r2c"); launch_pfa_z<T>(stream, pfa, tw, mesh_p, spec_p, 0, nb, (long)nreal, (long)nspec); }
      { TIMED("dft_y_fwd"); launch_pfa_y<T>(stream, pfa, tw, spec_p, 0, nb, (long)nspec); }
      { TIMED("dft_x_kspace"); launch_pfa_x_conv<T>(stream, pfa, tw, spec_p, tabs, Ed, slot, nb, (long)nspec); }
      { TIMED("dft_y_inv"); launch_pfa_y<T>(stream, pfa, tw, spec_p, 1, nb, (long)nspec); }
      { TIMED("dft_z_c2r"); launch_pfa_z<T>(stream, pfa, tw, mesh_p, spec_p, 1, nb, (long)nreal, (long)nspec); }
      return;
    }
    const T* tw = dft_tw.as<T>();
    { TIMED("dft_z_r2c"); launch_dft_z<T>(stream, K, tw, mesh_p, spec_p, 0, nb, (long)nreal, (long)nspec); }
    { TIMED("dft_y_fwd"); launch_dft_y<T>(stream, K, tw, spec_p, 0, nb, (long)nspec); }
    { TIMED("dft_x_kspace");
      if (mix) launch_dft_x_mix<T>(stream, K, tw, spec_p, tabs, *mix, (long)nspec, Ed, slot);
      else launch_dft_x_conv<T>(stream, K, tw, spec_p, tabs, Ed, slot, nb, (long)nspec); }
    { TIMED("dft_y_inv"); launch_dft_y<T>(stream, K, tw, spec_p, 1, nb, (long)nspec); }
    { TIMED("dft_z_c2r"); launch_dft_z<T>(stream, K, tw, mesh_p, spec_p, 1, nb, (long)nreal, (long)nspec); }
  }

  void run_plan(const char* label, rocfft_plan plan, void* in, void* out) {
    TIMED(label);
    FFT_TRY(rocfft_execution_info_set_stream(info_f, stream));
    void* i[1] = {in};
// ... 122 lines not shown
    for (int nb = 0; nb < 16; ++nb) {
      int idx = ((nb - 1) % ns + ns) % ns;
      t.mm[nb] = (T)(mS[idx] - 1.0);
      double p = pS ? pS[idx] : 0.0;
      t.p[nb] = (T)p;
      t.w0[nb] = (T)(1.0 / (std::exp((p - 1e-3) / 1e-5) + 1.0));
    }
    return t;
  }

  const T* stage_in(DevBuf& b, const void* p, size_t n, int on_device) {
    if (!p) return nullptr;
    if (on_device) return reinterpret_cast<const T*>(p);
    b.need(n * sizeof(T));
    HIP_TRY(hipMemcpyAsync(b.p, p, n * sizeof(T), hipMemcpyHostToDevice, stream));
    return b.as<T>();
  }

  void ensure_bins(int na) { ensure_bins(na, bins, bin_cells, bin_sorted); }
  void ensure_bins(int na, BinScratch& b, DevBuf& cells, DevBuf& sorted) {
    const int dims[3] = {nloc0(), K[1], K[2]};
    const BrickGrid bg = make_bricks(dims);
    cells.need(sizeof(int) * 3 * (size_t)(bg.ncell + 1));
    sorted.need(sizeof(int) * 8 * (size_t)na);
    bin_scan.need(spread_scan_bytes(bg.ncell));
    if (b.cell_start != cells.as<int>() || b.cursor != cells.as<int>() + (bg.ncell + 1))
      b.counters_zero = false;
    b.cell_start = cells.as<int>();
    b.cursor = cells.as<int>() + (bg.ncell + 1);
    b.fillcur = cells.as<int>() + 2 * (size_t)(bg.ncell + 1);
    b.sorted = sorted.as<int>();
    b.scan_tmp = bin_scan.p;
    b.scan_bytes = bin_scan.bytes;
  }

  void spread_sites(int n, const Site<T>* rows, int lp, const RecipGeom<T>& g, T* mesh_p, const int4* bases = nullptr, int nb = 1,
                    int reuse_bins = 0) {
    const int rc = launch_spread<T>(stream, n, rows, lp, g, bins, mesh_p, nullptr, bases, nb, reuse_bins);
    if (rc != 0) throw Err{ADMP_E_HIP, std::string("launch_spread: ") + hipGetErrorString((hipError_t)rc)};
  }

  struct Eval {
    const T* pos = nullptr; const T* Ql = nullptr; const T* pol = nullptr; const T* thole = nullptr;
    T* U = nullptr;
    Box<T> bx; RecipGeom<T> g; ScaleTab<T> tab;
    int n_home = 0; const int* home = nullptr;
    const int4* bases = nullptr;
    bool active = false;
  } ev;
  const int* pair_rows() const { return snranks > 1 ? sl.rows : nbr.order; }

  int stage_begin(const void* pos_, const double* box, const void* Ql_, const void* pol_, const void* thole_, int ns,
                  const double* mS, const double* pS, void* U_) {
    ARG_CHECK(have_top && have_ewald && have_pairs, "topology, ewald parameters and pairs must be set first");
    ARG_CHECK(pos_ && box && Ql_, "null argument");
    if (lpol) ARG_CHECK(pol_ && thole_ && U_ && pS, "polarizable handle needs pol, tholes, pScales and U_inout");
    const int na = top.na;
    double inv[9], vol;
    ++eval_seq;
    ff_done = nullptr;
    ensure_mesh();
    ev.bx = make_box(box, inv, &vol);
    ev.g = make_geom(inv);
    ev.tab = make_tab(ns, mS, pS);
    ensure_gtab(box, inv, vol, 1);
    ev.pos = reinterpret_cast<const T*>(pos_);
    ev.Ql = reinterpret_cast<const T*>(Ql_);
    ev.pol = lpol ? reinterpret_cast<const T*>(pol_) : nullptr;
    ev.thole = lpol ? reinterpret_cast<const T*>(thole_) : nullptr;
    ev.U = lpol ? reinterpret_cast<T*>(U_) : nullptr;
    const T* U_first = lpol && U_src_now ? reinterpret_cast<const T*>(U_src_now) : ev.U;
    U_src_now = nullptr;
    sites.need(sizeof(Site<T>) * (size_t)na);
    pot.need(9 * (size_t)na * sizeof(T));
    energies_d.need(2 * E_WORDS * sizeof(double));
    if (energies_d.p != energies_seen) { energies_seen = energies_d.p; other_clean = false; }
    if (lpol) {
      fld_pair.need(3 * (size_t)na * sizeof(T));
      fld_recip.need(3 * (size_t)na * sizeof(T));
      field.need(3 * (size_t)na * sizeof(T));
    }
    ensure_bins(na);
    bases_d.need(sizeof(int4) * (size_t)na);
    if (other_clean) {
      ehalf ^= 1;
    } else {
      ehalf = 0;
      HIP_TRY(hipMemsetAsync(energies_d.p, 0, E_WORDS * sizeof(double), stream));
    }
    other_clean = false;
    fmax_clean = true;
    for (bool& c : slot_clean) c = true;
    static const bool subset_on = env_flag("ADMP_SLAB_SUBSET", true);
    if (snranks > 1 && subset_on && slab_sites_na == na && slab_sites_ptr == sites.p && !cls_pending && have_pairs) {
      { TIMED("atom_bases"); launch_atom_bases<T>(stream, na, ev.pos, ev.g, bases_d.as<int4>()); }
      ev.bases = bases_d.as<int4>();
      cls_sites_na = na;
      ++cls_quiet;
      const bool tracked = lpol && sl.prev_na == na;
      decompose();
      {
        TIMED("prepare_sites");
        const int* lists[2] = {sl.home, sl.imp.as<int>()};
        const int counts[2] = {sl.n_home, sl.n_imp};
        for (int k = 0; k < 2; ++k)
          launch_prepare_sites<T>(stream, top, ev.pos, ev.Ql, U_first, ev.pol, ev.thole, ev.bx, sites.as<Site<T>>(),
                                  k == 0 ? energies_d.as<double>() + (size_t)(ehalf ^ 1) * E_WORDS : nullptr, ev.g, nullptr,
                                  nullptr, nullptr, nbr.cls, cls_flags_dev(), rq_p(), U_first != ev.U ? ev.U : nullptr, lists[k],
                                  counts[k]);
      }
      other_clean = true;
      if (tracked) exchange_migrants();
      if (lpol) exchange_U(0);
      ev.active = true;
      cut_pass();
      return ev.n_home;
    }
    {
      TIMED("prepare_sites");
      const bool have_list = act_n >= 0 && act_top_na == na && act_d.p;
      const bool want_act = lpol && snranks == 1 && !(keep_pol_sites && have_list);
      act_fresh = want_act;
      if (want_act) { act_d.need(sizeof(int) * (size_t)na); act_n = -1; act_top_na = na; ++act_gen; }
      if (cls_pending && have_pairs && cls_sites_na == na && !nbr_src) {
        unprune();
        if (!nbr.cls) HIP_TRY(hipMalloc(&nbr.cls, sizeof(int) * (size_t)na));
        launch_site_classes<T>(stream, na, sites.as<Site<T>>(), nbr.cls);
        apply_classes();
        order_rows();
      }
      cls_pending = false;
      cls_sites_na = na;
      ++cls_quiet;
      launch_prepare_sites<T>(stream, top, ev.pos, ev.Ql, U_first, ev.pol, ev.thole, ev.bx, sites.as<Site<T>>(),
                              energies_d.as<double>() + (size_t)(ehalf ^ 1) * E_WORDS, ev.g, bases_d.as<int4>(),
                              want_act ? act_d.as<int>() : nullptr, want_act ? nact_dev() : nullptr, nbr.cls,
                              cls_flags_dev(), rq_p(), U_first != ev.U ? ev.U : nullptr);
      ev.bases = bases_d.as<int4>();
      if (!nbr.cls && have_pairs && !nbr_src && !cls_first_done) {
        cls_first_done = true;
        int flags = 0;
        HIP_TRY(hipMemcpyAsync(&flags, cls_flags_dev(), sizeof(int), hipMemcpyDeviceToHost, stream));
        HIP_TRY(hipStreamSynchronize(stream));
        if (flags & CLS_BETTER) {
          unprune();
          HIP_TRY(hipMalloc(&nbr.cls, sizeof(int) * (size_t)na));
          launch_site_classes<T>(stream, na, sites.as<Site<T>>(), nbr.cls);
          apply_classes();
          order_rows();
          HIP_TRY(hipMemsetAsync(cls_flags_dev(), 0, sizeof(int), stream));
        }
      }
    }
    other_clean = true;
    if (snranks > 1) {
      slab_sites_na = na; slab_sites_ptr = sites.p;
      const bool tracked = lpol && sl.prev_na == na;
      decompose();
      if (tracked) exchange_migrants();
      if (lpol) exchange_U(0);
    } else {
      ev.n_home = na;
      ev.home = nullptr;
    }
    ev.active = true;
    cut_pass();
    return ev.n_home;
  }
  void cut_pass() {
    cut_on = cutoff > 0.0;
    if (!cut_on) return;
    const size_t na = (size_t)top.na, entries = (size_t)std::max<int64_t>(nbr.cap, 1);
    cut_end.need(sizeof(int) * na);
    cut_col.need(sizeof(int) * entries);
    cut_nbr = nbr;
    cut_nbr.col = cut_col.as<int>();
    cut_nbr.rowend = cut_end.as<int>();
    if (lpol) {
      cut_iend.need(sizeof(int) * na);
      cut_icol.need(sizeof(int) * entries);
      cut_ind.beg = nbr.rowptr; cut_ind.end = cut_iend.as<int>(); cut_ind.col = cut_icol.as<int>();
      cut_ind.cap = (int64_t)entries; cut_ind.na_cap = (int)na;
    }
    TIMED("cut_table");
    const int rc = build_cut_table<T>(stream, ev.n_home, pair_rows(), nbr, sites.as<Site<T>>(), ev.bx, cutoff,
                                      cut_end.as<int>(), cut_col.as<int>(), lpol ? cut_iend.as<int>() : nullptr,
                                      lpol ? cut_icol.as<int>() : nullptr);
    if (rc != 0) throw Err{ADMP_E_HIP, std::string("build_cut_table: ") + hipGetErrorString((hipError_t)rc)};
  }

  void need_eval() { ARG_CHECK(ev.active, "internal: no evaluation in progress"); }

  void stage_spread(T* mesh_p) {
    need_eval();
    TIMED("spread");
    int rc = launch_spread<T>(stream, ev.n_home, sites.as<Site<T>>(), lpol, ev.g, bins, mesh_p, ev.home, ev.bases);
    if (rc != 0) throw Err{ADMP_E_HIP, std::string("launch_spread: ") + hipGetErrorString((hipError_t)rc)};
  }
  unsigned long long* fmax_word() { return reinterpret_cast<unsigned long long*>(Ed_cur() + E_FMAX); }
  void launch_field_finish_only() {
    need_eval();
    if (!fmax_clean) HIP_TRY(hipMemsetAsync(fmax_word(), 0, sizeof(unsigned long long), stream));
    fmax_clean = false;
    { TIMED("field_finish");
      launch_field_finish<T>(stream, ev.n_home, sites.as<Site<T>>(), ev.pol, ev.U, fld_pair.as<T>(), fld_recip.as<T>(),
                             (T)kappa, field.as<T>(), fmax_word(), ev.home); }
    reduce_check_word(fmax_word());
  }
  void check_mono_inputs(bool use_mono) {
    if (use_mono && !rq_d.p) throw Err{ADMP_E_STATE, "charge-only pair forms requested without the compact site rows"};
  }
  hipStream_t side = nullptr;
  hipEvent_t ev_fork = nullptr, ev_join = nullptr;
  bool side_busy = false;
  bool overlap_ok() const {
    static const int mx = env_int("ADMP_OVERLAP_MAX", 200000);
    static const int mn = env_int("ADMP_OVERLAP_MIN", 4096);
    return side_stream_on && snranks == 1 && top.na <= mx && top.na >= mn;
  }
  void after_error() override {
    if (side) (void)hipStreamSynchronize(side);
// ... 97 lines not shown
  }
  void launch_finish_only(T* grad_p, T* dQl, bool with_field_finish = false) {
    need_eval();
    if (fin_fused) { fin_fused = false; return; }
    FieldFin<T> ff;
    if (with_field_finish) {
      if (!fmax_clean) HIP_TRY(hipMemsetAsync(fmax_word(), 0, sizeof(unsigned long long), stream));
      fmax_clean = false;
      ff.pol = ev.pol; ff.Ucart = ev.U; ff.fld_pair = fld_pair.as<T>(); ff.fld_recip = fld_recip.as<T>();
      ff.kappa = (T)kappa; ff.field = field.as<T>(); ff.fmax_bits = fmax_word();
    }
    { TIMED("finish");
      launch_finish<T>(stream, top, ev.pos, ev.bx, sites.as<Site<T>>(), ev.pol, ev.U, lpol, (T)kappa, pot.as<T>(), grad_p,
                       dQl, Ed_cur(), ev.home, ev.n_home, ff, snranks > 1 ? sl.bits.as<int>() : nullptr); }
    if (snranks > 1 && grad_p) exchange_grad(grad_p);
  }
  enum { E_PARTS_SUM = -1 };
  int* nact_dev() { return reinterpret_cast<int*>(Ed_cur() + E_NACT); }
  DevBuf rq_d;
  RQ4<T>* rq_p() {
    rq_d.need(sizeof(RQ4<T>) * (size_t)top.na);
    return rq_d.as<RQ4<T>>();
  }
  int* cls_flags_dev() { return nact_dev() + 1; }
  int cls_sites_na = -1;
  bool cls_first_done = false;
  const int* act_list() const { return snranks > 1 ? sl.act : act_d.as<int>(); }
  const int* nact_arg() { return snranks == 1 && act_fresh ? nact_dev() : nullptr; }
  int nact_rows() const { return snranks > 1 ? sl.n_act : (act_fresh ? top.na : act_n); }
  int nact_known() const { return snranks > 1 ? sl.n_act : act_n; }
  void nact_seen() {
    if (snranks > 1 || !act_fresh) return;
    int n = 0;
    std::memcpy(&n, &Eh[E_NACT], sizeof(n));
    act_n = n;
    act_fresh = false;
    act_tmp.need(sizeof(int) * (size_t)(n > 0 ? n : 1));
    int rc = sort_ints(stream, act_d.as<int>(), act_tmp.as<int>(), n, &scan_scratch.p, &scan_bytes);
    if (rc != 0) throw Err{ADMP_E_HIP, std::string("sort_ints: ") + hipGetErrorString((hipError_t)rc)};
  }
  PairFieldArgs<T> pair_field_common(int kind, int n_rows) {
    PairFieldArgs<T> a;
    a.kind = kind; a.na = n_rows; a.sites = sites.as<Site<T>>(); a.box = ev.bx; a.tab = ev.tab; a.kappa = (T)kappa;
    a.fld = fld_pair.as<T>(); a.rows = act_list();
    return a;
  }
  PairFieldArgs<T> pair_field_args() {
    const NbrTable& nb = wnbr();
    PairFieldArgs<T> a = pair_field_common(1, nact_rows());
    a.rowptr = nb.rowptr; a.rowend = nb.rowend; a.col = nb.col;
    a.n_dev = nact_arg(); a.cls_flags = cls_flags_dev(); a.rq = rq_d.as<RQ4<T>>(); a.tholes = ev.thole;
    return a;
  }
  PairFieldArgs<T> pair_field_ind_args(int n_act) {
    const IndTable& it = wind();
    PairFieldArgs<T> a = pair_field_common(2, n_act);
    a.rowptr = it.beg; a.rowend = it.end; a.col = it.col;
    return a;
  }
  void first_pair_field() {
    check_mono_inputs(true);
    const PairFieldArgs<T> a = pair_field_args();
    TIMED("pair_field");
    launch_pair_field<T>(stream, a);
  }
  void first_gather_field(const FieldFin<T>& ff) {
    join_side();
    TIMED("gather_field");
    launch_gather_field<T>(stream, nact_rows(), sites.as<Site<T>>(), ev.g, mesh.as<T>(), fld_recip.as<T>(), act_list(), 1,
                           nact_arg(), nullptr, ff);
  }
  double scf_check(int* n_act) {
    if (ff_done == fmax_word()) ff_done = nullptr;
    else launch_field_check(next_check_word());
    double dummy[4];
    const double fmax = read_energies(E_SCF_RECIP, dummy, false);
    nact_seen();
    *n_act = nact_known();
    return fmax;
  }
  void scf_jacobi(int n_act, const unsigned long long* gate = nullptr, double gate_min = 0.0, double relax = 1.0) {
    if (n_act > 0) {
      isites.need(sizeof(Site<T>) * (size_t)n_act);
      TIMED("jacobi_update");
      launch_jacobi_delta<T>(stream, n_act, act_list(), ev.pol, field.as<T>(), ev.U, sites.as<Site<T>>(),
                             isites.as<Site<T>>(), gate, gate_min, relax);
    }
    if (snranks > 1) exchange_U(1);
  }
  const unsigned long long* ff_done = nullptr;
  static int fuse_ff_max() { static const int v = env_int("ADMP_FUSE_FF_MAX", 16384); return v; }
  bool fuse_ok() const { return top.na <= fuse_ff_max() && snranks == 1 && !ev.home; }
  FieldFin<T> field_epilogue(unsigned long long* word) {
    FieldFin<T> ff;
    if (!word || !fuse_ok()) return ff;
    ff.pol = ev.pol; ff.Ucart = ev.U; ff.fld_pair = fld_pair.as<T>(); ff.kappa = (T)kappa;
    ff.field = field.as<T>(); ff.fmax_bits = word; ff.sites = sites.as<Site<T>>();
    ff_done = word;
    return ff;
  }
  unsigned long long* next_check_word() {
    if (!fmax_clean) HIP_TRY(hipMemsetAsync(fmax_word(), 0, sizeof(unsigned long long), stream));
    fmax_clean = false;
    return fmax_word();
  }
  void launch_field_check(unsigned long long* word) {
    if (ff_done == word) { ff_done = nullptr; return; }
    ff_done = nullptr;
    if (nact_rows() > 0) {
      TIMED("field_finish");
      launch_field_finish<T>(stream, nact_rows(), sites.as<Site<T>>(), ev.pol, ev.U, fld_pair.as<T>(), fld_recip.as<T>(),
                             (T)kappa, field.as<T>(), word, act_list(), nact_arg());
    }
    reduce_check_word(word);
  }
  size_t nreal_local() const { return (size_t)nloc0() * K[1] * K[2]; }
  bool scf_increment(int n_act, unsigned long long* check_word = nullptr,
                     const std::function<void()>& extra_side = nullptr, bool field_from_total_phi = false,
                     T* full_grad = nullptr, bool no_field = false) {
    if (n_act <= 0 && snranks == 1) {
      if (extra_side) on_side(extra_side);
      return false;
    }
    const bool first = side_first();
    PairFieldArgs<T> fr;
    bool ride = false;
    auto side_work = [&] {
      if (!ride && !no_field)
        on_side([&] {
          TIMED("pair_field_ind");
          launch_pair_field_ind<T>(stream, fr);
        });
      if (extra_side) on_side(extra_side);
    };
    if (!cut_on && (ind_nbr_gen != nbr_gen || ind_act_gen != act_gen)) {
      TIMED("ind_table");
      int rc = build_ind_table<T>(stream, top.na, nbr, sites.as<Site<T>>(), ind);
      if (rc != 0) throw Err{ADMP_E_HIP, std::string("build_ind_table: ") + hipGetErrorString((hipError_t)rc)};
      ind_nbr_gen = nbr_gen; ind_act_gen = act_gen;
    }
    fr = pair_field_ind_args(n_act);
    ride = !no_field && rider_ok() && field_rider<T>(fr);
    if (first) side_work();
    const size_t nreal = nreal_local();
    mesh2.need(nreal * sizeof(T));
    const bool fused = spread_fused(n_act);
    if (fused) { if (!first) side_work(); }
    else { TIMED("spread_ind");
      ensure_bins(std::max(n_act, 1), bins_ind, bin_cells_ind, bin_sorted_ind);
      const bool reuse = ind_bins_eval == eval_seq && ind_bins_n == n_act && ind_bins_gen == act_gen &&
                         ind_bins_at == bins_ind.cell_start;
      int rc = launch_spread<T>(stream, n_act, isites.as<Site<T>>(), 1, ev.g, bins_ind, mesh2.as<T>(), nullptr, nullptr, 1,
                                reuse ? 1 : 0, 0);
      ind_bins_eval = eval_seq; ind_bins_n = n_act; ind_bins_gen = act_gen; ind_bins_at = bins_ind.cell_start;
      if (rc != 0) throw Err{ADMP_E_HIP, std::string("launch_spread: ") + hipGetErrorString((hipError_t)rc)}; }
    if (!first && !fused) side_work();
    const PlaneSpread<T> sp = plane_spread(n_act, isites.as<Site<T>>(), 1, nullptr);
    PairFullArgs<T> pr;
    const bool full_rides = full_grad && pair_full_rider(pr, full_grad);
    const bool added = convolve(mesh2.as<T>(), spec.as<T>(), gtab_cur, E_SCRATCH, mesh.as<T>(), nullptr, fused ? &sp : nullptr,
                                ride ? &fr : nullptr, full_rides ? &pr : nullptr);
    join_side();
    if (!field_from_total_phi && !no_field) {
      TIMED("gather_field_ind");
      launch_gather_field<T>(stream, n_act, isites.as<Site<T>>(), ev.g, mesh2.as<T>(), fld_recip.as<T>(), nullptr, 1, nullptr,
                             act_list(), check_word ? field_epilogue(check_word) : FieldFin<T>()); }
    if (!added) { TIMED("mesh_add"); launch_mesh_add<T>(stream, (long)nreal, mesh.as<T>(), mesh2.as<T>()); }
    return full_rides;
  }

  double read_energies(int recip_slot, double* E, bool want_sum = true) {
    if (!Eh) HIP_TRY(hipHostMalloc(reinterpret_cast<void**>(&Eh), E_WORDS * sizeof(double), hipHostMallocDefault));
    const bool summed = snranks > 1 && want_sum;
    if (summed) {
      TIMED("comm_energies");
      launch_energy_pack(stream, Ed_cur(), recip_slot, Ed_cur() + E_RED);
      c_all_reduce(Ed_cur() + E_RED, 4, ADMP_T_F64, ADMP_OP_SUM, ADMP_TAG_ENERGIES);
    }
    HIP_TRY(hipMemcpyAsync(Eh, Ed_cur(), E_WORDS * sizeof(double), hipMemcpyDeviceToHost, stream));
    HIP_TRY(hipStreamSynchronize(stream));
    {
      int w[2];
      std::memcpy(w, &Eh[E_NACT], sizeof(w));
      cls_seen(w[1]);
    }
    if (summed) {
      for (int k = 0; k < 4; ++k) E[k] = Eh[E_RED + k];
      return Eh[E_FMAX];
    }
    E[0] = Eh[E_REAL]; E[1] = recip_slot >= 0 ? Eh[recip_slot] : 0.0; E[2] = Eh[E_SELF]; E[3] = Eh[E_PEN];
    for (int k = 0; k < E_PARTS; ++k) E[0] += Eh[E_RPARTS + k];
    if (recip_slot == E_PARTS_SUM) {
      double e = 0.0;
      for (int k = 0; k < E_PARTS; ++k) e += Eh[E_SLOTS + k];
      E[1] = e;
    }
    return Eh[E_FMAX];
  }
  void stage_finish(T* grad_p, T* dQl, int recip_slot, double* E) {
    launch_finish_only(grad_p, dQl);
    read_energies(recip_slot, E);
    ev.active = false;
  }

  template <class F>
  void recip_pass(int slot, F&& side_work, const PairFieldArgs<T>* rider = nullptr, const PairFullArgs<T>* prider = nullptr) {
    need_eval();
    const bool fused = spread_fused(ev.n_home);
    const bool first = side_first() || fused;
    if (first) side_work();
    if (!fused) stage_spread(mesh.as<T>());
    if (!first) side_work();
    if (!slot_clean[slot]) HIP_TRY(hipMemsetAsync(Ed_cur() + slot, 0, sizeof(double), stream));
    slot_clean[slot] = false;
    const PlaneSpread<T> sp = plane_spread(ev.n_home, sites.as<Site<T>>(), lpol, ev.bases);
    convolve(mesh.as<T>(), spec.as<T>(), gtab_cur, slot, nullptr, nullptr, fused ? &sp : nullptr, rider, prider);
  }
  void recip_pass_pair_full(int slot, T* grad_p, T* fld_out = nullptr) {
    PairFullArgs<T> pr;
    if (pair_full_rider(pr, grad_p, fld_out)) recip_pass(slot, [] {}, nullptr, &pr);
    else recip_pass(slot, [&] { on_side([&] { stage_pair_full(grad_p, fld_out); }); });
  }
  void recip_pass(int slot) { recip_pass(slot, [] {}); }
  void recip_pass_first_field(int slot) {
    if (rider_ok()) {
      check_mono_inputs(true);
      const PairFieldArgs<T> fr = pair_field_args();
      if (field_rider<T>(fr)) {
        recip_pass(slot, [] {}, &fr);
        return;
      }
    }
    recip_pass(slot, [&] { on_side([&] { first_pair_field(); }); });
  }

  struct PmeIo {
    const T *pos = nullptr, *Ql = nullptr, *pol = nullptr, *thole = nullptr;
    T *U = nullptr, *dpos = nullptr, *dQl = nullptr;
    T* gbuf = nullptr;
    double* E = nullptr;
// ... 1486 lines not shown

int admp_slab_configure(admp_handle* h, int rank, int nranks) {
  return guarded(h, [&](EngineBase& e) {
    ARG_CHECK(nranks >= 1 && nranks <= kSlabMaxRanks && rank >= 0 && rank < nranks, "bad rank / nranks (at most 28 ranks)");
    e.srank = rank; e.snranks = nranks;
    if (nranks > 1) e.aspc_off();
  });
}
int admp_slab_info(admp_handle* h, int64_t* out11) {
  return guarded(h, [&](EngineBase& e) { ARG_CHECK(out11, "null"); e.slab_info(out11); });
}
int admp_set_comm(admp_handle* h, const admp_comm* comm) {
  return guarded(h, [&](EngineBase& e) {
    if (!comm) { e.have_comm = false; e.comm = admp_comm{}; return; }
    ARG_CHECK(comm->all_reduce && comm->all_to_all_v && comm->shift, "communicator with a missing callback");
    e.comm = *comm;
    e.have_comm = true;
  });
}
int admp_set_comm_rccl(admp_handle* h, admp_rccl* c) {
  return guarded(h, [&](EngineBase& e) {
    if (!c) { e.rccl = nullptr; if (!e.comm.all_reduce) e.have_comm = false; return; }
    ARG_CHECK(rccl_device(c) == e.device, "the communicator was created on another device");
    ARG_CHECK(rccl_nranks(c) <= kSlabMaxRanks, "at most 28 slab ranks");
    e.rccl = c;
    e.srank = rccl_rank(c); e.snranks = rccl_nranks(c);
    if (e.snranks > 1) e.aspc_off();
    e.have_comm = true;
  });
}
int admp_set_dipole_source(admp_handle* h, const void* U_init) {
  return guarded(h, [&](EngineBase& e) { e.U_src = U_init; });
}
int admp_set_cutoff(admp_handle* h, double rc) {
  return guarded(h, [&](EngineBase& e) {
    ARG_CHECK(rc >= 0.0, "negative cutoff");
    e.cutoff = rc;
  });
}
int admp_scf_aspc(admp_handle* h, int order, int n_corrector, double omega) {
  return guarded(h, [&](EngineBase& e) {
    ARG_CHECK(aspc_args_ok(order, n_corrector, omega),
              "order must be -1 (off) or 0..4, n_corrector 1..6, omega <= 0 (Kolafa's value) or in (0, 1]");
    if (order >= 0) {
      if (!e.have_ewald || !e.lpol) throw Err{ADMP_E_STATE, "admp_scf_aspc needs a polarizable handle (admp_set_ewald with lpol)"};
      if (e.snranks > 1) throw Err{ADMP_E_STATE, "admp_scf_aspc: not on a slab-decomposed handle"};
    }
    e.aspc.configure(order, n_corrector, omega);
    e.aspc_dirty = false;
    for (int64_t& c : e.aspc_calls) c = 0;
    e.aspc_resid = 0.0;
  });
}
int admp_scf_aspc_reset(admp_handle* h) {
  return guarded(h, [&](EngineBase& e) { e.aspc.drop(); });
}
int admp_scf_aspc_info(admp_handle* h, int64_t* out8, double* out2) {
  return guarded(h, [&](EngineBase& e) {
    ARG_CHECK(out8 && out2, "null");
    out8[0] = e.aspc.order(); out8[1] = e.aspc.on() ? e.aspc.n_corrector() : 0; out8[2] = e.aspc.count();
    for (int k = 0; k < 3; ++k) out8[3 + k] = e.aspc_calls[k];
    out8[6] = out8[7] = 0;
    out2[0] = e.aspc.omega(); out2[1] = e.aspc_resid;
  });
}
int admp_scf_stats(admp_handle* h, int64_t* out8, int reset) {
  return guarded(h, [&](EngineBase& e) {
    ARG_CHECK(out8, "null");
    for (int k = 0; k < 8; ++k) { out8[k] = e.scf_stats[k]; if (reset) e.scf_stats[k] = 0; }
  });
}
int admp_xpass_stats(admp_handle* h, int64_t* out2, int reset) {
  return guarded(h, [&](EngineBase& e) {
    ARG_CHECK(out2, "null");
    for (int k = 0; k < 2; ++k) { out2[k] = e.xpass_stats[k]; if (reset) e.xpass_stats[k] = 0; }
  });
}
int admp_plane_mfma_stats(admp_handle* h, int64_t* out2, int reset) {
  return guarded(h, [&](EngineBase& e) {
    ARG_CHECK(out2, "null");
    for (int k = 0; k < 2; ++k) { out2[k] = e.plane_mfma_stats[k]; if (reset) e.plane_mfma_stats[k] = 0; }
  });
}
int admp_plane_mfma_stats4(admp_handle* h, int64_t* out4, int reset) {
  return guarded(h, [&](EngineBase& e) {
    ARG_CHECK(out4, "null");
    for (int k = 0; k < 4; ++k) { out4[k] = e.plane_mfma_stats4[k]; if (reset) e.plane_mfma_stats4[k] = 0; }
  });
}
int admp_mesh_convolve(admp_handle* h, const double* box, int which, void* mesh_inout, int on_device, double* E_out,
                       int32_t* info16) {
  return guarded(h, [&](EngineBase& e) { e.mesh_convolve(box, which, mesh_inout, on_device, E_out, info16); });
}
int admp_slab_mesh_convolve(admp_handle* h, const double* box, int which, void* mesh_inout, int on_device, double* E_out,
                            int32_t* info16) {
  return guarded(h, [&](EngineBase& e) { e.slab_mesh_convolve(box, which, mesh_inout, on_device, E_out, info16); });
}
int admp_pair_real(admp_handle* h, const void* positions, const double* box, const void* Q_local, const void* pol,
                   const void* tholes, int n_scales, const double* mScales, const double* pScales, const void* U,
                   const void* F, int which, int flags, int on_device, double* E_out, void* grad, void* pot, void* fld,
                   int32_t* info4) {
  return guarded(h, [&](EngineBase& e) {
    e.pair_real(positions, box, Q_local, pol, tholes, n_scales, mScales, pScales, U, F, which, flags, on_device, E_out, grad,
                pot, fld, info4);
  });
}
int admp_mesh_spread(admp_handle* h, const void* positions, const double* box, const void* Q_local, const void* pol,
                     const void* tholes, const void* U, int which, int flags, int on_device, void* mesh_out, int32_t* info8) {
  return guarded(h, [&](EngineBase& e) {
    e.mesh_spread(positions, box, Q_local, pol, tholes, U, which, flags, on_device, mesh_out, info8);
  });
}
int admp_mesh_gather(admp_handle* h, const void* positions, const double* box, const void* Q_local, const void* pol,
                     const void* tholes, const void* U, const void* phi_in, int which, int on_device, double* E_out, void* pot,
                     void* grad, void* fld, int32_t* info4) {
  return guarded(h, [&](EngineBase& e) {
    e.mesh_gather(positions, box, Q_local, pol, tholes, U, phi_in, which, on_device, E_out, pot, grad, fld, info4);
  });
}
int admp_pair_rider_stats(admp_handle* h, int64_t* out2, int reset) {
  return guarded(h, [&](EngineBase& e) {
    ARG_CHECK(out2, "null");
    for (int k = 0; k < 2; ++k) { out2[k] = e.pair_rider_stats[k]; if (reset) e.pair_rider_stats[k] = 0; }
  });
}
int admp_slab_home(admp_handle* h, int32_t* home_out, int* n_home, int* n_import) {
  return guarded(h, [&](EngineBase& e) { e.slab_home(home_out, n_home, n_import); });
}
int admp_slab_lists(admp_handle* h, int n_atoms, int nranks, int32_t* owner, int32_t* bits, int32_t* home, int32_t* rows,
                    int32_t* act, int32_t* imp, int32_t* exp, int32_t* mig_in, int32_t* mig_out, int64_t* counts) {
  return guarded(h, [&](EngineBase& e) {
    e.slab_lists(n_atoms, nranks, owner, bits, home, rows, act, imp, exp, mig_in, mig_out, counts);
  });
}

int admp_profile_enable(admp_handle* h, int on) {
  return guarded(h, [&](EngineBase& e) { e.prof.collect(e.stream); e.prof.on = on != 0; });
}
int admp_profile_filter(admp_handle* h, const char* label) {
  return guarded(h, [&](EngineBase& e) { e.prof.only = label ? label : ""; });
}
int admp_profile_reset(admp_handle* h) {
  return guarded(h, [&](EngineBase& e) { e.prof.reset(e.stream); });
}
int admp_profile_count(admp_handle* h) {
  if (!h || !h->eng) return ADMP_E_ARG;
  try { h->eng->prof.collect(h->eng->stream); } catch (const Err& e) { h->err = e.msg; return e.code; }
  return (int)h->eng->prof.labels.size();
}
int admp_profile_entry(admp_handle* h, int idx, const char** label, double* total_ms, int64_t* launches) {
  return guarded(h, [&](EngineBase& e) {
    e.prof.collect(e.stream);
    ARG_CHECK(idx >= 0 && idx < (int)e.prof.labels.size(), "profile index out of range");
    if (label) *label = e.prof.labels[idx].c_str();
    if (total_ms) *total_ms = e.prof.total_ms[idx];
    if (launches) *launches = e.prof.count[idx];
  });
}

}
```

### admp_amd/csrc/launch.h

```cpp
#pragma once
#include <hip/hip_runtime.h>
#include <stdint.h>

#include <initializer_list>

#include "env.h"
#include "frame_math.h"
#include "brick_plan.h"
#include "con_plan.h"
#include "mol_plan.h"
#include "mts_plan.h"
#include "pfa_maps.h"
#include "pme_math.h"
#include "scf_aspc.h"
#include "spline_math.h"

namespace admp {

template <class T>
struct ScaleTab {
  T mm[16];
  T p[16];
  T w0[16];
};

struct NbrTable {
  int* rowptr = nullptr;
  int* col = nullptr;
  int* rowend = nullptr;
  int64_t n_half = 0;
  int64_t cap = 0;
  int* order = nullptr;
  int* cls = nullptr;
  int* order_plain = nullptr;
  int* col_alt = nullptr;
  int64_t cap_alt = 0;
  int* deg = nullptr;
  int deg_na = 0;
  unsigned char* built = nullptr;
  void free_all() {
    for (int** p : {&rowptr, &col, &order, &cls, &order_plain, &col_alt, &deg})
      if (*p) { (void)hipFree(*p); *p = nullptr; }
    if (built) { (void)hipFree(built); built = nullptr; }
    n_half = cap = cap_alt = 0; deg_na = 0;
  }
};
constexpr int kRowWindow = 1024;
constexpr int kColMask = 0x0fffffff;
constexpr int kColMono = (int)0x80000000u;
constexpr int kNbMask = 7;
__host__ __device__ inline int col_nb(int c) { return (c >> 28) & kNbMask; }
enum { CLS_STALE = 1 , CLS_BETTER = 2  };

struct Topology {
  int na = 0;
  int* axis_type = nullptr;
  int* axis_idx = nullptr;
  int* excl_ptr = nullptr;
  int* excl_col = nullptr;
  int* excl_nb = nullptr;
  int* inv_ptr = nullptr;
  int* inv_idx = nullptr;
  int* grp_ptr = nullptr;
  int ngroups = 0;
  int* rows_blk = nullptr;
  int nrowblk = 0;
  int* grp_of = nullptr;
  int* gath_blk = nullptr;
  int ngathblk = 0;
};
constexpr int kFinishBlock = 256;
constexpr int kGatherRun = 32;
template <class T>
struct FinishArgs {
  const T* pol = nullptr;
  T kappa = 0;
  T* dQlocal = nullptr;
  double* energies = nullptr;
  int want_grad = 1;
};
constexpr int kMaxGroup = 4;

enum { E_REAL = 0, E_RECIP = 1, E_SELF = 2, E_PEN = 3, E_NACT = 4 ,
       E_SCRATCH = 5 , E_SCF_RECIP = 6, E_FMAX = 7 ,
       E_FMAX1 = 8 , E_CHAIN = 6,
       E_SLOTS = E_FMAX1 + E_CHAIN,
       E_PARTS = 64 ,
       E_RED = E_SLOTS + E_PARTS ,
       E_RPARTS = E_RED + 4 ,
       E_WORDS = E_RPARTS + E_PARTS  };

template <class T>
struct FieldFin {
  const T* pol = nullptr;
  const T* Ucart = nullptr;
  const T* fld_pair = nullptr;
  const T* fld_recip = nullptr;
  T kappa = 0;
  T* field = nullptr;
  unsigned long long* fmax_bits = nullptr;
  const Site<T>* sites = nullptr;
};
template <class T>
void launch_site_classes(hipStream_t st, int na, const Site<T>* sites, int* cls);
template <class T>
void launch_prepare_sites(hipStream_t st, const Topology& top, const T* pos, const T* Qlocal, const T* Ucart,
                          const T* pol, const T* thole, const Box<T>& box, Site<T>* sites,
                          double* zero_next ,
                          const RecipGeom<T>& g, int4* bases ,
                          int* act_list = nullptr ,
                          int* act_count = nullptr ,
                          const int* cls = nullptr ,
                          int* cls_flags = nullptr ,
                          RQ4<T>* rq = nullptr ,
                          T* Ucopy = nullptr ,
                          const int* list = nullptr , int nlist = 0 );
template <class T>
void launch_local_frames(hipStream_t st, const Topology& top, const T* pos, const Box<T>& box, T* out );
template <class T>
void launch_field_finish(hipStream_t st, int na, const Site<T>* sites, const T* pol, const T* Ucart, const T* fld_pair,
                         const T* fld_recip, T kappa, T* field, unsigned long long* fmax_bits, const int* list,
                         const int* n_dev = nullptr);
template <class T>
void launch_jacobi_delta(hipStream_t st, int n_act, const int* act, const T* pol, const T* field, T* Ucart, Site<T>* sites,
                         Site<T>* isites, const unsigned long long* gate = nullptr ,
                         double gate_min = 0.0 ,
                         double relax = 1.0 );
template <class T>
struct AspcSets {
  int n = 0;
  const T* U[kAspcMaxSets] = {};
  double B[kAspcMaxSets] = {};
};
template <class T>
void launch_aspc_predict(hipStream_t st, long n_words, const AspcSets<T>& h, T* out);
template <class T>
void launch_finish(hipStream_t st, const Topology& top, const T* pos, const Box<T>& box, const Site<T>* sites,
                   const T* pol, const T* Ucart, int lpol, T kappa, T* pot, T* grad, T* dQlocal, double* energies,
                   const int* list, int nlist,
                   const FieldFin<T>& ff = FieldFin<T>(),
                   const int* slab_bits = nullptr );
template <class T>
void launch_scalar_sites(hipStream_t st, int na, const T* pos, const T* vals, int stride, int chan, double self_coef,
                         Site<T>* sites, double* energies);
template <class T>
void launch_scale_add(hipStream_t st, int na, const T* vals, int stride, int chan, const T* v, T* grad, int nch = 1);
struct SelfCoefs {
  double c[3] = {0, 0, 0};
};
template <class T>
void launch_scalar_sites_batch(hipStream_t st, int na, const T* pos, const T* vals, int stride, int nch,
                               const double* self_coefs, Site<T>* sites, double* energies,
                               const RecipGeom<T>* g = nullptr ,
                               int4* bases = nullptr );
int dft_tile_cols(int N);
template <class T>
struct DftTabs {
  const T* p[3] = {nullptr, nullptr, nullptr};
};
template <class T>
bool dft_zy_fits(const int K[3]);
template <class T>
struct PlaneSpread {
  int na = 0, lpol = 0;
  const Site<T>* sites = nullptr;
  const int4* bases = nullptr;
  RecipGeom<T> g;
};
template <class T>
bool dft_zy_spread_fits(const int K[3], int na);
template <class T>
bool launch_dft_zy(hipStream_t st, const int K[3], const T* tw, T* mesh, T* spec, int inverse, int nb = 1, long mesh_stride = 0,
                   long spec_stride = 0, T* accum = nullptr, const PlaneSpread<T>* sp = nullptr ,
                   int* mfma_share = nullptr );
template <class T>
bool launch_dft_z(hipStream_t st, const int K[3], const T* tw, T* mesh, T* spec, int inverse, int nb = 1,
                  long mesh_stride = 0, long spec_stride = 0,
                  T* accum = nullptr );
template <class T>
void launch_dft_y(hipStream_t st, const int K[3], const T* tw, T* spec, int inverse, int nb = 1,
                  long spec_stride = 0);
template <class T>
void launch_dft_x_conv(hipStream_t st, const int K[3], const T* tw, T* spec, const DftTabs<T>& tabs, double* energies,
                       int slot, int nb = 1, long spec_stride = 0);
template <class T>
void launch_dft_x_circ(hipStream_t st, const int K[3], T* spec, const T* ctab, double* energies, int slot);
template <class T>
void launch_ctab(hipStream_t st, const int K[3], const T* gtab, T* ctab, int* uneven);

struct PfaPlan {
  PfaAxis ax[3];
  int Khp;
  int tw_off[3];
  const int* ptab[3];
};
bool pfa_split(int N, PfaAxis* out);
void pfa_forms(const PfaPlan& p, size_t w, int out[9]);
template <class T>
void launch_pfa_z(hipStream_t st, const PfaPlan& p, const T* tw, T* mesh, T* spec, int inverse, int nb = 1, long mesh_stride = 0,
                  long spec_stride = 0);
template <class T>
void launch_pfa_y(hipStream_t st, const PfaPlan& p, const T* tw, T* spec, int inverse, int nb = 1, long spec_stride = 0);
template <class T>
void launch_pfa_x_conv(hipStream_t st, const PfaPlan& p, const T* tw, T* spec, const DftTabs<T>& tabs, double* energies, int slot,
                       int nb = 1, long spec_stride = 0);

bool fftx_usable(int N);
template <class T>
void launch_fftx_conv(hipStream_t st, const int K[3], const T* tw, T* spec, const T* gtab, double* energies, int slot,
                      int khp = 0 ,
                      int ny = 0 );
template <class T>
void launch_fftx_conv_batch(hipStream_t st, const int K[3], const T* tw, T* spec, const DftTabs<T>& tabs, int nb,
                            long spec_stride , double* energies, int slot,
                            int khp = 0, int ny = 0);

struct IndTable {
  const int* beg = nullptr;
  int* end = nullptr;
  int* col = nullptr;
  int64_t cap = 0;
  int na_cap = 0;
};
template <class T>
struct PairFullArgs {
  int on = 0, na = 0;
  const int* rowptr = nullptr;
  const int* rowend = nullptr;
  const int* col = nullptr;
  const Site<T>* sites = nullptr;
  Box<T> box;
  ScaleTab<T> tab;
  T kappa = 0;
  T* grad = nullptr;
  T* pot = nullptr;
  double* energies = nullptr;
  const int* rows = nullptr;
  T* fld = nullptr;
  unsigned nblocks = 0, grid = 0;
  int use_mono = 0;
  const int* cls_flags = nullptr;
  const RQ4<T>* rq = nullptr;
  const T* tholes = nullptr;
};
template <class T>
struct PairFieldArgs {
  int kind = 0, na = 0;
  const int* rowptr = nullptr;
  const int* rowend = nullptr;
  const int* col = nullptr;
// ... 310 lines not shown
```

### admp_amd/pme.py

```python
import contextlib
import ctypes
import math
import warnings

import numpy as np
import torch

from . import _lib, settings
from ._device import HipForceBase

DIELECTRIC = 1389.35455846
DEFAULT_THOLE_WIDTH = 0.3


def setup_ewald_parameters(rc, ethresh, box):
    box = np.asarray(box.detach().cpu() if isinstance(box, torch.Tensor) else box, dtype=np.float64)
    kappa = math.sqrt(-math.log(2 * ethresh)) / rc
    K1 = math.ceil(2 * kappa * box[0, 0] / 3 / ethresh ** 0.2)
    K2 = math.ceil(2 * kappa * box[1, 1] / 3 / ethresh ** 0.2)
    K3 = math.ceil(2 * kappa * box[2, 2] / 3 / ethresh ** 0.2)
    if settings.FFT_FRIENDLY_MESH:
        K1, K2, K3 = (next_smooth(int(k)) for k in (K1, K2, K3))
    return kappa, int(K1), int(K2), int(K3)

# ... 307 lines not shown
        pos = self._real(positions, (na, 3))
        Q = self._pad_Q(Q_local)
        boxa, _ = self._harr('box', box, 9)
        mSa, ns = self._harr('mS', mScales)
        pol_t = th_t = U = pS = None
        if self.lpol:
            pol_t, th_t = self._real(pol, (na,)), self._real(tholes, (na,))
            pS, _ = self._harr('pS', pScales, ns)
            U = self._real(self.U_ind, (na, 3))
        E = self._out_E
        dbox = (ctypes.c_double * 9)()
        P = self._ptr
        _lib.check(self._h, self._L.admp_pme_box_grad(self._h, P(pos), boxa, P(Q), P(pol_t), P(th_t), ns, mSa, pS, P(U), E,
                                                      dbox), 'admp_pme_box_grad')
        self.energy_parts = tuple(E)
        return np.float64(E[0] + E[1] + E[2] + E[3]), np.array(dbox[:], dtype=np.float64).reshape(3, 3)

    def get_pscale_gradient(self, positions, box, pairs, Q_local, pol, tholes, mScales, pScales, dScales, U_init=None):
        if not self.lpol:
            raise RuntimeError('get_pscale_gradient needs lpol=True')
        with self._not_a_step():
            self.get_energy(positions, box, pairs, Q_local, pol, tholes, mScales, pScales, dScales, U_init=U_init)
        self._use_current_stream()
        na = self.n_atoms
        pos = self._real(positions, (na, 3))
        Q = self._pad_Q(Q_local)
        mS = self._host64(mScales)
        pS = self._host64(pScales, len(mS))
        out = (ctypes.c_double * len(mS))()
        pol_t, th_t, U = self._real(pol, (na,)), self._real(tholes, (na,)), self._real(self.U_ind, (na, 3))
        rc = self._L.admp_pscale_grad(self._h, self._ptr(pos), _lib.darr(self._host64(box, 9)), self._ptr(Q),
                                      self._ptr(pol_t), self._ptr(th_t), len(mS), _lib.darr(mS), _lib.darr(pS), self._ptr(U),
                                      out)
        _lib.check(self._h, rc, 'admp_pscale_grad')
        return np.array(out[:], dtype=np.float64)

    def get_mscale_gradient(self, positions, box, pairs, Q_local, mScales):
        return self._mscale_gradient(0, positions, box, pairs, self._pad_Q(Q_local), 9, len(self._host64(mScales)))

    def set_aspc(self, order=2, n_corrector=1, omega=None):
        if not self.lpol:
            raise RuntimeError('set_aspc needs lpol=True')
        if order is None:
            order, n_corrector, omega = -1, 1, None
        if isinstance(order, bool) or isinstance(n_corrector, bool) or int(order) != order or int(n_corrector) != n_corrector:
            raise ValueError('set_aspc: order and n_corrector must be integers')
        if omega is not None and not (0.0 < float(omega) <= 1.0):
            raise ValueError('set_aspc: omega must lie in (0, 1], got %r' % (omega,))
        rc = self._L.admp_scf_aspc(self._h, int(order), int(n_corrector), 0.0 if omega is None else float(omega))
        if rc == _lib.E_ARG:
            raise ValueError('set_aspc: ' + self._L.admp_last_error(self._h).decode())
        _lib.check(self._h, rc, 'admp_scf_aspc')

    def reset_aspc(self):
        _lib.check(self._h, self._L.admp_scf_aspc_reset(self._h), 'admp_scf_aspc_reset')

    def aspc_info(self):
        out8, out2 = (ctypes.c_int64 * 8)(), (ctypes.c_double * 2)()
        _lib.check(self._h, self._L.admp_scf_aspc_info(self._h, out8, out2), 'admp_scf_aspc_info')
        return {'order': int(out8[0]), 'n_corrector': int(out8[1]), 'stored': int(out8[2]), 'fixed': int(out8[3]),
                'warmup': int(out8[4]), 'fallback': int(out8[5]), 'omega': float(out2[0]), 'residual': float(out2[1])}

    @contextlib.contextmanager
    def _not_a_step(self):
        opt = self._L.admp_set_option
        _lib.check(self._h, opt(self._h, _lib.OPT_ASPC_HOLD, 1), 'admp_set_option')
        try:
            yield
        finally:
            _lib.check(self._h, opt(self._h, _lib.OPT_ASPC_HOLD, 0), 'admp_set_option')

    def scf_stats(self, reset=False):
        out = (ctypes.c_int64 * 8)()
        _lib.check(self._h, self._L.admp_scf_stats(self._h, out, 1 if reset else 0), 'admp_scf_stats')
        keys = ('plain', 'speculative', 'speculative_failed', 'chained', 'chained_too_short', 'chained_too_long',
                'wasted_increments', 'jacobi_steps')
        return dict(zip(keys, (int(v) for v in out)))

    def xpass_stats(self, reset=False):
        out = (ctypes.c_int64 * 2)()
        _lib.check(self._h, self._L.admp_xpass_stats(self._h, out, 1 if reset else 0), 'admp_xpass_stats')
        return {'circulant': int(out[0]), 'transforms': int(out[1])}

    def plane_mfma_stats(self, reset=False):
        out = (ctypes.c_int64 * 2)()
        _lib.check(self._h, self._L.admp_plane_mfma_stats(self._h, out, 1 if reset else 0), 'admp_plane_mfma_stats')
        out4 = (ctypes.c_int64 * 4)()
        _lib.check(self._h, self._L.admp_plane_mfma_stats4(self._h, out4, 1 if reset else 0), 'admp_plane_mfma_stats4')
        return {'matrix_share': int(out[0]), 'vector': int(out[1]), 'inverse_share': int(out4[2]), 'inverse_vector': int(out4[3])}

    def pair_rider_stats(self, reset=False):
        out = (ctypes.c_int64 * 2)()
        _lib.check(self._h, self._L.admp_pair_rider_stats(self._h, out, 1 if reset else 0), 'admp_pair_rider_stats')
        return {'rode': int(out[0]), 'own_launch': int(out[1])}

    def pair_real(self, positions, box, pairs, Q_local, mScales, pol=None, tholes=None, pScales=None, U=None, which=0,
                  flags=1, field=None):
        self._use_current_stream()
        L, h, na = self._L, self._h, self.n_atoms
        self.set_pairs(pairs)
        pos = self._real(positions, (na, 3))
        Q = self._pad_Q(Q_local)
        mS = self._host64(mScales)
        pol_t = th_t = U_t = pS = F_t = None
        if self.lpol:
            pol_t, th_t, U_t = self._real(pol, (na,)), self._real(tholes, (na,)), self._real(U, (na, 3))
            pS = _lib.darr(self._host64(pScales, len(mS)))
            F_t = self._real(field, (na, 3)) if field is not None else None

        def new(k):
            return torch.empty((na, k), dtype=self._dtype, device=self._device)
        grad, pot = (new(3), new(9)) if which == 0 else (None, None)
        fld = new(3) if self.lpol else None
        E = ctypes.c_double(0.0)
        info = (ctypes.c_int * 4)()
        P = self._ptr
        rc = L.admp_pair_real(h, P(pos), _lib.darr(self._host64(box, 9)), P(Q), P(pol_t), P(th_t), len(mS), _lib.darr(mS), pS,
                              P(U_t), P(F_t), int(which), int(flags), 1, ctypes.byref(E), P(grad), P(pot), P(fld), info)
        _lib.check(h, rc, 'admp_pair_real')
        return {'E': E.value, 'grad': grad, 'pot': pot, 'fld': fld, 'info': tuple(int(v) for v in info)}

    def _mesh_inputs(self, positions, pairs, Q_local, pol, tholes, U):
        self._use_current_stream()
        na = self.n_atoms
        self.set_pairs(pairs)
        pol_t = th_t = U_t = None
        if self.lpol:
            pol_t, th_t, U_t = self._real(pol, (na,)), self._real(tholes, (na,)), self._real(U, (na, 3))
        return self._real(positions, (na, 3)), self._pad_Q(Q_local), pol_t, th_t, U_t

    def mesh_spread(self, positions, box, pairs, Q_local, pol=None, tholes=None, U=None, which=0, flags=1):
        pos, Q, pol_t, th_t, U_t = self._mesh_inputs(positions, pairs, Q_local, pol, tholes, U)
        out = torch.empty((self.K1, self.K2, self.K3), dtype=self._dtype, device=self._device)
        info = (ctypes.c_int * 8)()
        P = self._ptr
        rc = self._L.admp_mesh_spread(self._h, P(pos), _lib.darr(self._host64(box, 9)), P(Q), P(pol_t), P(th_t), P(U_t),
                                      int(which), int(flags), 1, P(out), info)
        _lib.check(self._h, rc, 'admp_mesh_spread')
        v = [int(x) for x in info]
        return out, {'form': _lib.SPREAD_FORMS[v[0]], 'bricks': tuple(v[1:4]), 'tight': v[4],
                     'path': _lib.MESH_PATHS[v[5]] if v[5] >= 0 else None, 'records': v[6]}

    def mesh_gather(self, positions, box, pairs, Q_local, phi, pol=None, tholes=None, U=None, which=0):
        pos, Q, pol_t, th_t, U_t = self._mesh_inputs(positions, pairs, Q_local, pol, tholes, U)
        na = self.n_atoms
        phi_t = self._real(phi, (self.K1, self.K2, self.K3))

        def new(k):
            return torch.empty((na, k), dtype=self._dtype, device=self._device)
        grad, pot = (new(3), new(9)) if which == 0 else (None, None)
        fld = new(3) if self.lpol else None
        E = ctypes.c_double(0.0)
        info = (ctypes.c_int * 4)()
        P = self._ptr
        rc = self._L.admp_mesh_gather(self._h, P(pos), _lib.darr(self._host64(box, 9)), P(Q), P(pol_t), P(th_t), P(U_t),
                                      P(phi_t), int(which), 1, ctypes.byref(E), P(pot), P(grad), P(fld), info)
        _lib.check(self._h, rc, 'admp_mesh_gather')
        return {'E': E.value, 'pot': pot, 'grad': grad, 'fld': fld, 'info': tuple(int(v) for v in info)}

    def optimize_Uind(self, positions, box, pairs, Q_local, pol, tholes, mScales, pScales, dScales, U_init=None,
                      maxiter=None, thresh=None):
        if not self.lpol:
            raise RuntimeError('optimize_Uind needs lpol=True')
        r = self._evaluate(positions, box, pairs, Q_local, mScales, pol, tholes, pScales, dScales, U_init,
                           want_grad=False, maxiter=maxiter, thresh=thresh)
        self._warn_unconverged(r)
# ... 2 lines not shown
```

### include/admp_hip.h

```cpp
#ifndef ADMP_HIP_H
#define ADMP_HIP_H

#include <stdint.h>

#ifdef __cplusplus
extern "C" {
#endif

typedef struct admp_handle admp_handle;

enum {
  ADMP_OK = 0,
  ADMP_E_ARG = -1,
  ADMP_E_HIP = -2,
  ADMP_E_FFT = -3,
  ADMP_E_NOGPU = -4,
  ADMP_E_STATE = -5,
  ADMP_E_COMM = -6
};

const char* admp_version(void);

int admp_create(admp_handle** out, int device, int precision );
int admp_destroy(admp_handle* h);
// ... 80 lines not shown
int admp_md_bonded(admp_handle* h, const void* positions, const double* box, int n_bonds, const int32_t* bond_idx,
                   const void* bond_par, int n_angles, const int32_t* angle_idx, const void* angle_par, double* E_dev,
                   void* grad_inout);
int admp_md_kick_drift(admp_handle* h, int n_atoms, void* positions, void* velocities, const void* grad, const void* inv_mass,
                       double half_dt_acc, double dt, double* ekin_dev);
int admp_md_langevin(admp_handle* h, int n_atoms, void* positions, void* velocities, const void* grad, const void* inv_mass,
                     double half_dt_acc, double dt, double c1, double c2sq_kT_acc, uint64_t seed, uint64_t step,
                     double* ekin_dev);
int admp_md_random(admp_handle* h, int kind, int64_t n, uint64_t seed, uint64_t step, uint32_t stream, void* out);
int admp_md_bonded_box(admp_handle* h, const void* positions, const double* box, int n_bonds, const int32_t* bond_idx,
                       const void* bond_par, int n_angles, const int32_t* angle_idx, const void* angle_par, double* E_dev,
                       double* S_dev);
int admp_md_virial(admp_handle* h, int n_atoms, const void* positions, const void* velocities, const void* grad,
                   const void* inv_mass, uint64_t seed, uint64_t step, double* out_dev);
int admp_md_scale(admp_handle* h, int n_atoms, void* positions, void* velocities, double mu);
int admp_md_mts_plan(admp_handle* h, int n_atoms, int n_bonds, const int32_t* bond_idx, const double* bond_par, int n_angles,
                     const int32_t* angle_idx, const double* angle_par, int tile_atoms);
int admp_md_mts_step(admp_handle* h, int n_atoms, void* positions, void* velocities, const void* grad_slow, const void* inv_mass,
                     const double* box, double half_dt_acc_outer, double dt_outer, int n_inner, double c1, double c2sq_kT_acc,
                     uint64_t seed, uint64_t outer_step, double* E_dev, void* grad_fast_out);
int admp_md_mts_info(admp_handle* h, int64_t* out8);
int admp_md_con_plan(admp_handle* h, int n_atoms, int n_constraints, const int32_t* pairs, const double* lengths, int tile_atoms);
int admp_md_con_step(admp_handle* h, int n_atoms, void* positions, void* velocities, const void* grad, const void* inv_mass,
                     const double* box, double half_dt_acc, double dt, double c1, double c2sq_kT_acc, uint64_t seed, uint64_t step,
                     double tolerance, int max_sweeps, int32_t* counters_dev);
int admp_md_con_kick(admp_handle* h, int n_atoms, const void* positions, void* velocities, const void* grad, const void* inv_mass,
                     const double* box, double half_dt_acc, double dt, double tolerance, int max_sweeps, double* ekin_dev,
                     int32_t* counters_dev);
int admp_md_con_project(admp_handle* h, int n_atoms, void* positions, const void* reference, const void* inv_mass, const double* box,
                        double tolerance, int max_sweeps, int32_t* counters_dev);
int admp_md_con_info(admp_handle* h, int64_t* out8);
int admp_md_mol_plan(admp_handle* h, int n_atoms, const int32_t* group_of, int tile_atoms);
int admp_md_mol_sums(admp_handle* h, int n_atoms, const void* positions, const void* velocities, const void* grad, const void* inv_mass,
                     const double* box, uint64_t seed, uint64_t step, double* out21_dev);
int admp_md_mol_scale(admp_handle* h, int n_atoms, void* positions, void* velocities, const void* inv_mass, const double* box,
                      double mu_minus_1, double inv_mu_minus_1);
int admp_md_mol_info(admp_handle* h, int64_t* out8);
int admp_md_fire_step(admp_handle* h, int n_atoms, void* positions, void* velocities, const void* grad, const void* inv_mass,
                      const double* params9, double ftol, uint64_t call, double* state16_dev);
int admp_md_vrescale(admp_handle* h, int n_atoms, void* velocities, const void* grad ,
                     const void* inv_mass, double half_dt_acc, int64_t n_dof, double kT_acc, double c, uint64_t seed, uint64_t step,
                     uint64_t call, double* state16_dev);

enum { ADMP_T_I32 = 0, ADMP_T_F32 = 1, ADMP_T_F64 = 2 };
enum { ADMP_OP_SUM = 0, ADMP_OP_MAX = 1 };
enum { ADMP_TAG_GHOST = 1, ADMP_TAG_TRANSPOSE = 2, ADMP_TAG_HALO_DIPOLES = 3, ADMP_TAG_HALO_GRADIENT = 4, ADMP_TAG_SCF_MAX = 5,
       ADMP_TAG_ENERGIES = 6 };
typedef struct admp_comm {
  void* ctx;
  int (*all_reduce)(void* ctx, void* buf, int64_t count, int dtype, int op, int tag);
  int (*all_to_all_v)(void* ctx, const void* send, const int64_t* send_counts, void* recv, const int64_t* recv_counts,
                      int dtype, int tag);
  int (*shift)(void* ctx, const void* send, void* recv, int64_t count, int dtype, int to_next, int tag);
} admp_comm;
int admp_slab_configure(admp_handle* h, int rank, int nranks);
int admp_set_comm(admp_handle* h, const admp_comm* comm);
int admp_slab_info(admp_handle* h, int64_t* out11);
typedef struct admp_rccl admp_rccl;
enum { ADMP_RCCL_ID_BYTES = 128, ADMP_RCCL_NTAGS = 8 };
int admp_rccl_unique_id(void* out128);
int admp_rccl_create(admp_rccl** out, int device, const void* id128, int rank, int nranks);
int admp_rccl_destroy(admp_rccl* c);
int admp_rccl_abort(admp_rccl* c);
int admp_rccl_stats(admp_rccl* c, int64_t* bytes_out, int64_t* calls_out, int reset);
int admp_rccl_all_reduce(admp_rccl* c, void* buf, int64_t count, int dtype , int op , void* hip_stream);
int admp_rccl_all_to_all_v(admp_rccl* c, const void* send, const int64_t* send_counts, void* recv, const int64_t* recv_counts,
                           int dtype, void* hip_stream);
int admp_rccl_shift(admp_rccl* c, const void* send, void* recv, int64_t count, int dtype, int to_next, void* hip_stream);
int admp_rccl_version(int* version);
const char* admp_rccl_last_error(void);
int admp_set_comm_rccl(admp_handle* h, admp_rccl* c);
int admp_slab_home(admp_handle* h, int32_t* home_out, int* n_home, int* n_import);
int admp_slab_lists(admp_handle* h, int n_atoms, int nranks, int32_t* owner, int32_t* bits, int32_t* home, int32_t* rows,
                    int32_t* act, int32_t* imp, int32_t* exp, int32_t* mig_in, int32_t* mig_out, int64_t* counts);

int admp_scf_stats(admp_handle* h, int64_t* out8, int reset);

int admp_scf_aspc(admp_handle* h, int order, int n_corrector, double omega);
int admp_scf_aspc_reset(admp_handle* h);
int admp_scf_aspc_info(admp_handle* h, int64_t* out8, double* out2);
int admp_xpass_stats(admp_handle* h, int64_t* out2, int reset);
int admp_plane_mfma_stats(admp_handle* h, int64_t* out2, int reset);
int admp_plane_mfma_stats4(admp_handle* h, int64_t* out4, int reset);
#define ADMP_MESH_INFO_WORDS 16
#define ADMP_MESH_PATH_ROCFFT 0
#define ADMP_MESH_PATH_FUSED_X 1
#define ADMP_MESH_PATH_DIRECT_LINES 2
#define ADMP_MESH_PATH_DIRECT_PLANES 3
#define ADMP_MESH_PATH_TWO_LEVEL 4
int admp_mesh_convolve(admp_handle* h, const double* box, int which, void* mesh_inout, int on_device, double* E_out,
                       int32_t* info16);
int admp_slab_mesh_convolve(admp_handle* h, const double* box, int which, void* mesh_inout, int on_device, double* E_out,
                            int32_t* info16);
int admp_pair_real(admp_handle* h, const void* positions, const double* box, const void* Q_local, const void* pol,
                   const void* tholes, int n_scales, const double* mScales, const double* pScales, const void* U,
                   const void* F, int which, int flags, int on_device, double* E_out, void* grad, void* pot, void* fld,
                   int32_t* info4);
#define ADMP_SPREAD_FORM_SCAN 0
#define ADMP_SPREAD_FORM_PLANES 1
#define ADMP_SPREAD_FORM_BRICKS 2
#define ADMP_SPREAD_FORM_PLANE_KERNEL 3
int admp_mesh_spread(admp_handle* h, const void* positions, const double* box, const void* Q_local, const void* pol,
                     const void* tholes, const void* U, int which, int flags, int on_device, void* mesh_out, int32_t* info8);
int admp_mesh_gather(admp_handle* h, const void* positions, const double* box, const void* Q_local, const void* pol,
                     const void* tholes, const void* U, const void* phi_in, int which, int on_device, double* E_out, void* pot,
                     void* grad, void* fld, int32_t* info4);
int admp_pair_rider_stats(admp_handle* h, int64_t* out2, int reset);

int admp_profile_enable(admp_handle* h, int on);
int admp_profile_filter(admp_handle* h, const char* label);
int admp_profile_reset(admp_handle* h);
int admp_profile_count(admp_handle* h);
int admp_profile_entry(admp_handle* h, int idx, const char** label, double* total_ms, int64_t* launches);

#ifdef __cplusplus
}
#endif
#endif
```

Before: 549.7 ns/day.

## Precompute per-atom B-spline records once per eval and reuse them in fused plane spread

Extra blocks of the prepare-sites kernel now compute per-atom, per-axis B-spline weights and derivatives into SplineRec buffers. The fused Z/Y plane-spread DFT kernel reads these records instead of recomputing splines for every plane block. On the induced-dipole SCF path it scans compact (atom, base) rows written by the Jacobi update, so it no longer re-reads the full bases array. This trades redundant spline arithmetic for extra global-memory traffic of about 60 doubles per atom and adds a stats counter.

```diff
diff --git a/admp_amd/_lib.py b/admp_amd/_lib.py
--- a/admp_amd/_lib.py
+++ b/admp_amd/_lib.py
@@ -79,6 +79,7 @@
     'admp_xpass_stats':(_i32, [_vp, _c.POINTER(_i64), _i32]),
     'admp_plane_mfma_stats': (_i32, [_vp, _c.POINTER(_i64), _i32]),
     'admp_plane_mfma_stats4': (_i32, [_vp, _c.POINTER(_i64), _i32]),
+    'admp_plane_spread_stats': (_i32, [_vp, _c.POINTER(_i64), _i32]),
     'admp_mesh_convolve': (_i32, [_vp, _dp, _i32, _vp, _i32, _dp, _ip]),
     'admp_slab_mesh_convolve': (_i32, [_vp, _dp, _i32, _vp, _i32, _dp, _ip]),
     'admp_slab_lists': (_i32, [_vp, _i32, _i32, _ip, _ip, _ip, _ip, _ip, _ip, _ip, _ip, _ip, _c.POINTER(_i64)]),
diff --git a/admp_amd/csrc/atom_kernels.hip b/admp_amd/csrc/atom_kernels.hip
--- a/admp_amd/csrc/atom_kernels.hip
+++ b/admp_amd/csrc/atom_kernels.hip
@@ -39,7 +39,17 @@
                                                               int* __restrict__ act_list, int* __restrict__ act_count,
                                                               const int* __restrict__ cls, int* __restrict__ cls_flags,
                                                               RQ4<T>* __restrict__ rq, T* __restrict__ Ucopy,
-                                                              const int* __restrict__ list, int nlist) {
+                                                              const int* __restrict__ list, int nlist,
+                                                              SplineRec<T>* __restrict__ recs, int rec_blk0) {
+  if (recs && (int)blockIdx.x >= rec_blk0) {
+    const int t = ((int)blockIdx.x - rec_blk0) * kAtomBlock + threadIdx.x, a = t / 3, d = t - 3 * a;
+    if (a < top.na) {
+      T r[3];
+      load3(pos, a, r);
+      spline_rec_fill_axis(g, r, d, recs[a]);
+    }
+    return;
+  }
   int i = blockIdx.x * kAtomBlock + threadIdx.x;
   if (zero_next && i < E_WORDS) zero_next[i] = 0.0;
   if (list) {
@@ -116,10 +126,12 @@
                                                              T* __restrict__ Ucart, Site<T>* __restrict__ sites,
                                                              Site<T>* __restrict__ isites,
                                                              const unsigned long long* __restrict__ gate,
-                                                             unsigned long long gate_bits, T relax) {
+                                                             unsigned long long gate_bits, T relax,
+                                                             const int4* __restrict__ bases, int2* __restrict__ xrows) {
   const int slot = blockIdx.x * kAtomBlock + threadIdx.x;
   if (slot >= n_act) return;
   const int i = act[slot];
+  if (xrows) xrows[slot] = make_int2(i, bases[i].x);
   const bool on = !gate || *gate >= gate_bits;
   const T s = on ? -pol[i] * T(1.0 / kDielectric) * relax : T(0);
   const T dx = field[3 * i] * s, dy = field[3 * i + 1] * s, dz = field[3 * i + 2] * s;
@@ -657,12 +669,14 @@
 void launch_prepare_sites(hipStream_t st, const Topology& top, const T* pos, const T* Qlocal, const T* Ucart,
                           const T* pol, const T* thole, const Box<T>& box, Site<T>* sites, double* zero_next,
                           const RecipGeom<T>& g, int4* bases, int* act_list, int* act_count, const int* cls,
-                          int* cls_flags, RQ4<T>* rq, T* Ucopy, const int* list, int nlist) {
+                          int* cls_flags, RQ4<T>* rq, T* Ucopy, const int* list, int nlist, SplineRec<T>* recs) {
   const int n = list ? nlist : top.na;
   if (n <= 0 && !zero_next) return;
-  k_prepare_sites<T><<<nblk(n > E_WORDS || !zero_next ? (n > 0 ? n : 1) : E_WORDS), kAtomBlock, 0, st>>>(
+  if (list || n <= 0) recs = nullptr;
+  const int nab = nblk(n > E_WORDS || !zero_next ? (n > 0 ? n : 1) : E_WORDS);
+  k_prepare_sites<T><<<nab + (recs ? nblk(3 * n) : 0), kAtomBlock, 0, st>>>(
       top, pos, Qlocal, Ucart, pol, thole, box, sites, zero_next, g, bases, list ? nullptr : act_list,
-      list ? nullptr : act_count, cls, cls_flags, rq, Ucopy, list, nlist);
+      list ? nullptr : act_count, cls, cls_flags, rq, Ucopy, list, nlist, recs, nab);
 }
 template <class T>
 void launch_site_classes(hipStream_t st, int na, const Site<T>* sites, int* cls) {
@@ -677,11 +691,13 @@
 }
 template <class T>
 void launch_jacobi_delta(hipStream_t st, int n_act, const int* act, const T* pol, const T* field, T* Ucart, Site<T>* sites,
-                         Site<T>* isites, const unsigned long long* gate, double gate_min, double relax) {
+                         Site<T>* isites, const unsigned long long* gate, double gate_min, double relax, const int4* bases,
+                         int2* xrows) {
   unsigned long long bits;
   std::memcpy(&bits, &gate_min, sizeof(bits));
   if (n_act > 0)
-    k_jacobi_delta<T><<<nblk(n_act), kAtomBlock, 0, st>>>(n_act, act, pol, field, Ucart, sites, isites, gate, bits, (T)relax);
+    k_jacobi_delta<T><<<nblk(n_act), kAtomBlock, 0, st>>>(n_act, act, pol, field, Ucart, sites, isites, gate, bits, (T)relax,
+                                                          bases, bases ? xrows : nullptr);
 }
 template <class T>
 void launch_aspc_predict(hipStream_t st, long n, const AspcSets<T>& h, T* out) {
@@ -755,12 +771,12 @@
                                              double*, const RecipGeom<T>*, int4*);                                      \
   template void launch_prepare_sites<T>(hipStream_t, const Topology&, const T*, const T*, const T*, const T*, const T*, \
                                         const Box<T>&, Site<T>*, double*, const RecipGeom<T>&, int4*, int*, int*,       \
-                                        const int*, int*, RQ4<T>*, T*, const int*, int);                                \
+                                        const int*, int*, RQ4<T>*, T*, const int*, int, SplineRec<T>*);                 \
   template void launch_site_classes<T>(hipStream_t, int, const Site<T>*, int*);                                         \
   template void launch_field_finish<T>(hipStream_t, int, const Site<T>*, const T*, const T*, const T*, const T*, T, T*,  \
                                        unsigned long long*, const int*, const int*);                                    \
   template void launch_jacobi_delta<T>(hipStream_t, int, const int*, const T*, const T*, T*, Site<T>*, Site<T>*,        \
-                                       const unsigned long long*, double, double);                                    \
+                                       const unsigned long long*, double, double, const int4*, int2*);                \
   template void launch_aspc_predict<T>(hipStream_t, long, const AspcSets<T>&, T*);                                      \
   template void launch_finish<T>(hipStream_t, const Topology&, const T*, const Box<T>&, const Site<T>*, const T*,        \
                                  const T*, int, T, T*, T*, T*, double*, const int*, int, const FieldFin<T>&, const int*);
diff --git a/admp_amd/csrc/dft_kernels.hip b/admp_amd/csrc/dft_kernels.hip
--- a/admp_amd/csrc/dft_kernels.hip
+++ b/admp_amd/csrc/dft_kernels.hip
@@ -331,7 +331,8 @@
 
 #ifdef ADMP_ZY_TRACE
 __device__ long long* g_zy_trace;
-#define ZY_TRACE(slot) do { if (threadIdx.x == 0) g_zy_trace[((blockIdx.z * gridDim.y + blockIdx.y) * gridDim.x + blockIdx.x) * 8 + (slot)] = wall_clock64(); } while (0)
+constexpr int kZyTraceSlots = 16;
+#define ZY_TRACE(slot) do { if (threadIdx.x == 0) g_zy_trace[((blockIdx.z * gridDim.y + blockIdx.y) * gridDim.x + blockIdx.x) * kZyTraceSlots + (slot)] = wall_clock64(); } while (0)
 #define ZY_TRACE_END(slot) do { __syncthreads(); ZY_TRACE(slot); } while (0)
 #else
 #define ZY_TRACE(slot) do {} while (0)
@@ -363,6 +364,43 @@
   const long n = spare / (long)(kZyW * sizeof(T) + 2 * sizeof(int));
   return n > kZyBlock / 3 ? kZyBlock / 3 : (int)n;
 }
+__device__ __forceinline__ void zy_spread_hit(int px, int bx, int id, int K0, unsigned short* hits, int* nhit) {
+  int a = px - bx;
+  if (a < 0) a += K0;
+  if (bx >= 0 && a < 6) hits[atomicAdd(nhit, 1)] = (unsigned short)(id | (a << 13));
+}
+template <class T>
+__device__ __forceinline__ void zy_spread_tasks(const T* wts, const int* ebase, int cnt, int N2, int N3, Cx<T>* p, T* x0, T* xn) {
+  const int H3 = (N3 - 1) / 2;
+  for (int task = threadIdx.x; task < cnt * 6; task += kZyBlock) {
+    const int e = task / 6, b = task - e * 6;
+    const T* w = wts + e * kZyW;
+    const T m1 = w[6 + b], d1 = w[12 + b], e1 = w[18 + b];
+    const T P0 = w[0] * m1 + w[1] * d1 + w[2] * e1;
+    const T P1 = w[3] * m1 + w[4] * d1;
+    const T P2 = w[5] * m1;
+    const int jb = wrap_add(ebase[2 * e], b, N2), bz = ebase[2 * e + 1];
+#pragma unroll
+    for (int c = 0; c < 6; ++c) {
+      const T v = P0 * w[24 + c] + P1 * w[30 + c] + P2 * w[36 + c];
+      const int jc = wrap_add(bz, c, N3);
+      T* dst;
+      if (jc == 0) dst = &x0[jb];
+      else if (jc <= H3) dst = &p[(jc - 1) * N2 + jb].re;
+      else if (2 * jc == N3) dst = &xn[jb];
+      else dst = &p[(N3 - 1 - jc) * N2 + jb].im;
+      atomicAdd(dst, v);
+    }
+  }
+}
+template <class T>
+__device__ __forceinline__ void zy_spread_close(int N2, int N3, Cx<T>* p) {
+  const int H3 = (N3 - 1) / 2;
+  for (int t = threadIdx.x; t < H3 * N2; t += kZyBlock) {
+    const Cx<T> ab = p[t];
+    p[t] = Cx<T>{ab.re + ab.im, ab.re - ab.im};
+  }
+}
 template <class T>
 __device__ __forceinline__ void zy_plane_spread(const PlaneSpread<T>& sp, int px, int N2, int N3, Cx<T>* p, T* x0, T* xn,
                                                 unsigned char* scratch, int SUB) {
@@ -372,6 +410,7 @@
   int* ebase = reinterpret_cast<int*>(wts + (size_t)SUB * kZyW);
   const int H3 = (N3 - 1) / 2;
   const Site<T>* sites = sp.sites + (size_t)blockIdx.y * sp.na;
+  ZY_TRACE(8);
   for (int t = threadIdx.x; t < H3 * N2; t += kZyBlock) p[t] = Cx<T>{T(0), T(0)};
   for (int t = threadIdx.x; t < 2 * N2; t += kZyBlock) x0[t] = T(0);
   const RecipGeom<T>& g = sp.g;
@@ -391,14 +430,11 @@
         }
       }
     }
-#pragma unroll
-    for (int r = 0; r < kZyScan; ++r) {
-      int a = px - bx[r];
-      if (a < 0) a += g.K[0];
-      if (bx[r] >= 0 && a < 6)
-        hits[atomicAdd(&s_nhit, 1)] = (unsigned short)((c0 + (int)threadIdx.x + r * kZyBlock) | (a << 13));
-    }
+    ZY_TRACE_END(9);
+#pragma unroll
+    for (int r = 0; r < kZyScan; ++r) zy_spread_hit(px, bx[r], c0 + (int)threadIdx.x + r * kZyBlock, g.K[0], hits, &s_nhit);
     __syncthreads();
+    ZY_TRACE(10);
     const int nhit = s_nhit;
     const int nsub = (nhit + SUB - 1) / SUB, per = nsub > 0 ? (nhit + nsub - 1) / nsub : 0;
     for (int sub = 0; sub < nhit; sub += per) {
@@ -438,33 +474,111 @@
         }
       }
       __syncthreads();
-      for (int task = threadIdx.x; task < cnt * 6; task += kZyBlock) {
-        const int e = task / 6, b = task - e * 6;
-        const T* w = wts + e * kZyW;
-        const T m1 = w[6 + b], d1 = w[12 + b], e1 = w[18 + b];
-        const T P0 = w[0] * m1 + w[1] * d1 + w[2] * e1;
-        const T P1 = w[3] * m1 + w[4] * d1;
-        const T P2 = w[5] * m1;
-        const int jb = wrap_add(ebase[2 * e], b, N2), bz = ebase[2 * e + 1];
-#pragma unroll
-        for (int c = 0; c < 6; ++c) {
-          const T v = P0 * w[24 + c] + P1 * w[30 + c] + P2 * w[36 + c];
-          const int jc = wrap_add(bz, c, N3);
-          T* dst;
-          if (jc == 0) dst = &x0[jb];
-          else if (jc <= H3) dst = &p[(jc - 1) * N2 + jb].re;
-          else if (2 * jc == N3) dst = &xn[jb];
-          else dst = &p[(N3 - 1 - jc) * N2 + jb].im;
-          atomicAdd(dst, v);
+      ZY_TRACE(11);
+      zy_spread_tasks<T>(wts, ebase, cnt, N2, N3, p, x0, xn);
+      __syncthreads();
+      ZY_TRACE(12);
+    }
+  }
+  zy_spread_close<T>(N2, N3, p);
+}
+
+template <class T>
+struct ZyScan { int bx[kZyScan], at[kZyScan]; };
+template <class T>
+__device__ __forceinline__ void zy_scan_load(const PlaneSpread<T>& sp, int c0, ZyScan<T>& s) {
+#pragma unroll
+  for (int r = 0; r < kZyScan; ++r) {
+    const int i = c0 + (int)threadIdx.x + r * kZyBlock;
+    s.bx[r] = -1000; s.at[r] = i;
+    if (i < sp.na) {
+      if (sp.xrows) { const int2 ax = sp.xrows[i]; s.at[r] = ax.x; s.bx[r] = ax.y; }
+      else s.bx[r] = sp.bases[i].x;
+    }
+  }
+}
+template <class T>
+__device__ __forceinline__ void zy_plane_spread_recs(const PlaneSpread<T>& sp, int px, int N2, int N3, Cx<T>* p, T* x0, T* xn,
+                                                     unsigned char* scratch, int SUB, Cx<T>* tw3, Cx<T>* tw2,
+                                                     const Cx<T>* __restrict__ tw3g, const Cx<T>* __restrict__ tw2g) {
+  __shared__ int s_nhit_r;
+  unsigned short* hits = reinterpret_cast<unsigned short*>(scratch);
+  T* wts = reinterpret_cast<T*>(hits + kZyScan * kZyBlock);
+  int* ebase = reinterpret_cast<int*>(wts + (size_t)SUB * kZyW);
+  const int H3 = (N3 - 1) / 2;
+  const Site<T>* sites = sp.xrows ? sp.asites : sp.sites + (size_t)blockIdx.y * sp.na;
+  const SplineRec<T>* recs = sp.recs;
+  const bool inc = sp.xrows != nullptr;
+  ZyScan<T> sc;
+  zy_scan_load(sp, 0, sc);
+  const int tid = threadIdx.x;
+  const Cx<T> t3 = tw3g[tid < N3 ? tid : 0], t2 = tw2g[tid < N2 ? tid : 0];
+  ZY_TRACE(8);
+  for (int t = threadIdx.x; t < H3 * N2; t += kZyBlock) p[t] = Cx<T>{T(0), T(0)};
+  for (int t = threadIdx.x; t < 2 * N2; t += kZyBlock) x0[t] = T(0);
+  if (tid < N3) tw3[tid] = t3;
+  if (tid < N2) tw2[tid] = t2;
+  for (int t = tid + kZyBlock; t < N3; t += kZyBlock) tw3[t] = tw3g[t];
+  for (int t = tid + kZyBlock; t < N2; t += kZyBlock) tw2[t] = tw2g[t];
+  const RecipGeom<T>& g = sp.g;
+  for (int c0 = 0; c0 < sp.na; c0 += kZyScan * kZyBlock) {
+    if (threadIdx.x == 0) s_nhit_r = 0;
+    if (c0 > 0) zy_scan_load(sp, c0, sc);
+    __syncthreads();
+    ZY_TRACE_END(9);
+#pragma unroll
+    for (int r = 0; r < kZyScan; ++r) zy_spread_hit(px, sc.bx[r], sc.at[r], g.K[0], hits, &s_nhit_r);
+    __syncthreads();
+    ZY_TRACE(10);
+    const int nhit = s_nhit_r;
+    const int nsub = (nhit + SUB - 1) / SUB, per = nsub > 0 ? (nhit + nsub - 1) / nsub : 0;
+    for (int sub = 0; sub < nhit; sub += per) {
+      const int cnt = min(per, nhit - sub);
+      if ((int)threadIdx.x < 3 * cnt) {
+        const int e = threadIdx.x / 3, part = threadIdx.x - 3 * e;
+        const int h = hits[sub + e], atom = h & 0x1fff;
+        const SplineRec<T>& rec = recs[atom];
+        T* w = wts + e * kZyW;
+        if (part == 0) {
+          const int a = h >> 13;
+          const T m0 = rec.w[spline_rec_m(0, a)], d0 = rec.w[spline_rec_d1(0, a)], e0 = rec.w[spline_rec_d2(0, a)];
+          const Site<T>& site = sites[atom];
+          T Q[9], c1[3], c2[6];
+          if (inc) {
+#pragma unroll
+            for (int k = 0; k < 9; ++k) Q[k] = T(0);
+            Q[1] += site.pad[0]; Q[2] += site.pad[1]; Q[3] += site.pad[2];
+          } else {
+#pragma unroll
+            for (int k = 0; k < 9; ++k) Q[k] = site.Q[k];
+            if (sp.lpol) { Q[1] += site.U[0]; Q[2] += site.U[1]; Q[3] += site.U[2]; }
+          }
+          fold_multipole(g, Q, c1, c2);
+          w[0] = Q[0] * m0 + c1[0] * d0 + c2[0] * e0;
+          w[1] = c1[1] * m0 + c2[3] * d0;
+          w[2] = c2[1] * m0;
+          w[3] = c1[2] * m0 + c2[4] * d0;
+          w[4] = c2[5] * m0;
+          w[5] = c2[2] * m0;
+        } else {
+          const int o = part == 1 ? 6 : 24;
+          const T* src = rec.w + kSplineRecAxisWords * part;
+          T v[kSplineRecAxisWords];
+#pragma unroll
+          for (int k = 0; k < kSplineRecAxisWords; ++k) v[k] = src[k];
+#pragma unroll
+          for (int k = 0; k < kSplineRecAxisWords; ++k) w[o + k] = v[k];
+          ebase[2 * e + part - 1] = rec.base[part];
         }
       }
       __syncthreads();
-    }
-  }
-  for (int t = threadIdx.x; t < H3 * N2; t += kZyBlock) {
-    const Cx<T> ab = p[t];
-    p[t] = Cx<T>{ab.re + ab.im, ab.re - ab.im};
-  }
+      ZY_TRACE(11);
+      zy_spread_tasks<T>(wts, ebase, cnt, N2, N3, p, x0, xn);
+      __syncthreads();
+      ZY_TRACE(12);
+    }
+  }
+  zy_spread_close<T>(N2, N3, p);
 }
 
 template <class T, int SIGN>
@@ -599,10 +713,14 @@
   const T* plane = mesh + blockIdx.y * mesh_stride + (long)blockIdx.x * N2 * N3;
   Cx<T>* out = spec + blockIdx.y * spec_stride + (long)blockIdx.x * N2 * Kh;
   ZY_TRACE(0);
-  for (int t = threadIdx.x; t < N3; t += kZyBlock) tw3[t] = tw3g[t];
-  for (int t = threadIdx.x; t < N2; t += kZyBlock) tw2[t] = tw2g[t];
+  if (!(SPREAD && sp.recs)) {
+    for (int t = threadIdx.x; t < N3; t += kZyBlock) tw3[t] = tw3g[t];
+    for (int t = threadIdx.x; t < N2; t += kZyBlock) tw2[t] = tw2g[t];
+  }
   if (SPREAD) {
-    zy_plane_spread<T>(sp, (int)blockIdx.x, N2, N3, p, x0, xn, dft_smem + L.b, zy_spread_sub<T>(N2, N3));
+    if (sp.recs)
+      zy_plane_spread_recs<T>(sp, (int)blockIdx.x, N2, N3, p, x0, xn, dft_smem + L.b, zy_spread_sub<T>(N2, N3), tw3, tw2, tw3g, tw2g);
+    else zy_plane_spread<T>(sp, (int)blockIdx.x, N2, N3, p, x0, xn, dft_smem + L.b, zy_spread_sub<T>(N2, N3));
   } else {
     for (int t = threadIdx.x; t < H3 * N2; t += kZyBlock) {
       const int l = t / H3, jj = t - l * H3;
diff --git a/admp_amd/csrc/engine.hip b/admp_amd/csrc/engine.hip
--- a/admp_amd/csrc/engine.hip
+++ b/admp_amd/csrc/engine.hip
@@ -70,6 +70,7 @@
   int64_t xpass_stats[2] = {0, 0};
   int64_t plane_mfma_stats[2] = {0, 0};
   int64_t plane_mfma_stats4[4] = {0, 0, 0, 0};
+  int64_t plane_spread_stats[2] = {0, 0};
   int64_t pair_rider_stats[2] = {0, 0};
   AspcRing aspc;
   int64_t aspc_calls[3] = {0, 0, 0};
@@ -454,6 +455,9 @@
   const int* ind_bins_at = nullptr;
   DevBuf dft_tw;
   DevBuf bases_d;
+  DevBuf spline_recs_d, xrows_d;
+  long recs_eval = -1, xrows_eval = -1;
+  int xrows_n = -1;
   bool use_dft = false;
   bool use_pfa = false;
   PfaPlan pfa;
@@ -854,8 +858,20 @@
   PlaneSpread<T> plane_spread(int n, const Site<T>* rows, int lp, const int4* bases) const {
     PlaneSpread<T> sp;
     sp.na = n; sp.lpol = lp; sp.sites = rows; sp.bases = bases; sp.g = ev.g;
+    if (bases && recs_ready() && n == top.na && rows == sites.as<Site<T>>()) sp.recs = spline_recs_d.as<SplineRec<T>>();
     return sp;
   }
+  bool recs_ready() const { return recs_eval == eval_seq && spline_recs_d.p; }
+  PlaneSpread<T> plane_spread_inc(int n_act) const {
+    PlaneSpread<T> sp = plane_spread(n_act, isites.as<Site<T>>(), 1, nullptr);
+    if (inc_recs(n_act) && xrows_eval == eval_seq && xrows_n == n_act) {
+      sp.recs = spline_recs_d.as<SplineRec<T>>();
+      sp.xrows = xrows_d.as<int2>();
+      sp.asites = sites.as<Site<T>>();
+    }
+    return sp;
+  }
+  bool inc_recs(int n_act) const { return recs_ready() && ev.bases && n_act > 0 && spread_fused(n_act); }
   bool rider_ok() const {
     static const bool on = env_flag("ADMP_FIELD_RIDER", true);
     return on && use_dft && !use_pfa && snranks == 1 && !overlap_ok();
@@ -921,6 +937,7 @@
       int mf = 0;
       if (planes && sp) { TIMED("dft_spread_zy_fwd"); launch_dft_zy<T>(stream, K, tw, mesh_p, spec_p, 0, 1, 0, 0, nullptr, sp, &mf); }
       else if (planes) { TIMED("dft_zy_fwd"); launch_dft_zy<T>(stream, K, tw, mesh_p, spec_p, 0, 1, 0, 0, nullptr, nullptr, &mf); }
+      if (planes && sp) ++plane_spread_stats[sp->recs ? 0 : 1];
       if (planes) { ++plane_mfma_stats[mf ? 0 : 1]; ++plane_mfma_stats4[mf ? 0 : 1]; }
       else {
         { TIMED("dft_z_r2c"); launch_dft_z<T>(stream, K, tw, mesh_p, spec_p, 0); }
@@ -1209,6 +1226,9 @@
     }
     ensure_bins(na);
     bases_d.need(sizeof(int4) * (size_t)na);
+    const bool want_recs = snranks == 1 && use_dft && !use_pfa && dft_zy_spread_fits<T>(K, na) &&
+                           env_flag("ADMP_PLANE_SPREAD_RECS", true);
+    if (want_recs) spline_recs_d.need(sizeof(SplineRec<T>) * (size_t)na);
     if (other_clean) {
       ehalf ^= 1;
     } else {
@@ -1262,8 +1282,10 @@
       launch_prepare_sites<T>(stream, top, ev.pos, ev.Ql, U_first, ev.pol, ev.thole, ev.bx, sites.as<Site<T>>(),
                               energies_d.as<double>() + (size_t)(ehalf ^ 1) * E_WORDS, ev.g, bases_d.as<int4>(),
                               want_act ? act_d.as<int>() : nullptr, want_act ? nact_dev() : nullptr, nbr.cls,
-                              cls_flags_dev(), rq_p(), U_first != ev.U ? ev.U : nullptr);
+                              cls_flags_dev(), rq_p(), U_first != ev.U ? ev.U : nullptr, nullptr, 0,
+                              want_recs ? spline_recs_d.as<SplineRec<T>>() : nullptr);
       ev.bases = bases_d.as<int4>();
+      if (want_recs) recs_eval = eval_seq;
       if (!nbr.cls && have_pairs && !nbr_src && !cls_first_done) {
         cls_first_done = true;
         int flags = 0;
@@ -1527,9 +1549,12 @@
   void scf_jacobi(int n_act, const unsigned long long* gate = nullptr, double gate_min = 0.0, double relax = 1.0) {
     if (n_act > 0) {
       isites.need(sizeof(Site<T>) * (size_t)n_act);
+      const bool xr = inc_recs(n_act);
+      if (xr) { xrows_d.need(sizeof(int2) * (size_t)n_act); xrows_eval = eval_seq; xrows_n = n_act; }
       TIMED("jacobi_update");
       launch_jacobi_delta<T>(stream, n_act, act_list(), ev.pol, field.as<T>(), ev.U, sites.as<Site<T>>(),
-                             isites.as<Site<T>>(), gate, gate_min, relax);
+                             isites.as<Site<T>>(), gate, gate_min, relax, xr ? ev.bases : nullptr,
+                             xr ? xrows_d.as<int2>() : nullptr);
     }
     if (snranks > 1) exchange_U(1);
   }
@@ -1600,7 +1625,7 @@
       ind_bins_eval = eval_seq; ind_bins_n = n_act; ind_bins_gen = act_gen; ind_bins_at = bins_ind.cell_start;
       if (rc != 0) throw Err{ADMP_E_HIP, std::string("launch_spread: ") + hipGetErrorString((hipError_t)rc)}; }
     if (!first && !fused) side_work();
-    const PlaneSpread<T> sp = plane_spread(n_act, isites.as<Site<T>>(), 1, nullptr);
+    const PlaneSpread<T> sp = plane_spread_inc(n_act);
     PairFullArgs<T> pr;
     const bool full_rides = full_grad && pair_full_rider(pr, full_grad);
     const bool added = convolve(mesh2.as<T>(), spec.as<T>(), gtab_cur, E_SCRATCH, mesh.as<T>(), nullptr, fused ? &sp : nullptr,
@@ -3253,6 +3278,12 @@
     for (int k = 0; k < 2; ++k) { out2[k] = e.plane_mfma_stats[k]; if (reset) e.plane_mfma_stats[k] = 0; }
   });
 }
+int admp_plane_spread_stats(admp_handle* h, int64_t* out2, int reset) {
+  return guarded(h, [&](EngineBase& e) {
+    ARG_CHECK(out2, "null");
+    for (int k = 0; k < 2; ++k) { out2[k] = e.plane_spread_stats[k]; if (reset) e.plane_spread_stats[k] = 0; }
+  });
+}
 int admp_plane_mfma_stats4(admp_handle* h, int64_t* out4, int reset) {
   return guarded(h, [&](EngineBase& e) {
     ARG_CHECK(out4, "null");
diff --git a/admp_amd/csrc/launch.h b/admp_amd/csrc/launch.h
--- a/admp_amd/csrc/launch.h
+++ b/admp_amd/csrc/launch.h
@@ -14,6 +14,7 @@
 #include "pme_math.h"
 #include "scf_aspc.h"
 #include "spline_math.h"
+#include "spline_rec.h"
 
 namespace admp {
 
@@ -114,7 +115,8 @@
                           int* cls_flags = nullptr ,
                           RQ4<T>* rq = nullptr ,
                           T* Ucopy = nullptr ,
-                          const int* list = nullptr , int nlist = 0 );
+                          const int* list = nullptr , int nlist = 0 ,
+                          SplineRec<T>* recs = nullptr );
 template <class T>
 void launch_local_frames(hipStream_t st, const Topology& top, const T* pos, const Box<T>& box, T* out );
 template <class T>
@@ -125,7 +127,9 @@
 void launch_jacobi_delta(hipStream_t st, int n_act, const int* act, const T* pol, const T* field, T* Ucart, Site<T>* sites,
                          Site<T>* isites, const unsigned long long* gate = nullptr ,
                          double gate_min = 0.0 ,
-                         double relax = 1.0 );
+                         double relax = 1.0 ,
+                         const int4* bases = nullptr ,
+                         int2* xrows = nullptr );
 template <class T>
 struct AspcSets {
   int n = 0;
@@ -166,6 +170,9 @@
   const Site<T>* sites = nullptr;
   const int4* bases = nullptr;
   RecipGeom<T> g;
+  const SplineRec<T>* recs = nullptr;
+  const int2* xrows = nullptr;
+  const Site<T>* asites = nullptr;
 };
 template <class T>
 bool dft_zy_spread_fits(const int K[3], int na);
diff --git a/admp_amd/csrc/spline_rec.h b/admp_amd/csrc/spline_rec.h
--- /dev/null
+++ b/admp_amd/csrc/spline_rec.h
@@ -0,0 +1,32 @@
+#pragma once
+#include "spline_math.h"
+
+namespace admp {
+
+constexpr int kSplineRecAxisWords = 18;
+template <class T>
+struct SplineRec {
+  int base[3];
+  int pad;
+  T w[3 * kSplineRecAxisWords];
+};
+ADMP_HD int spline_rec_m(int d, int p) { return kSplineRecAxisWords * d + p; }
+ADMP_HD int spline_rec_d1(int d, int p) { return kSplineRecAxisWords * d + 6 + p; }
+ADMP_HD int spline_rec_d2(int d, int p) { return kSplineRecAxisWords * d + 12 + p; }
+
+template <class T>
+ADMP_HD void spline_rec_fill_axis(const RecipGeom<T>& g, const T r[3], int d, SplineRec<T>& rec) {
+  int base;
+  T M[6], D1[6], D2[6], D3[6];
+  const T f = grid_ref(g, r, d, base);
+  bspline6(f, M, D1, D2, D3);
+  rec.base[d] = base;
+  if (d == 0) rec.pad = 0;
+  for (int p = 0; p < 6; ++p) {
+    rec.w[spline_rec_m(d, p)] = M[p];
+    rec.w[spline_rec_d1(d, p)] = D1[p];
+    rec.w[spline_rec_d2(d, p)] = D2[p];
+  }
+}
+
+}
diff --git a/admp_amd/pme.py b/admp_amd/pme.py
--- a/admp_amd/pme.py
+++ b/admp_amd/pme.py
@@ -413,6 +413,11 @@
         _lib.check(self._h, self._L.admp_xpass_stats(self._h, out, 1 if reset else 0), 'admp_xpass_stats')
         return {'circulant': int(out[0]), 'transforms': int(out[1])}
 
+    def plane_spread_stats(self, reset=False):
+        out = (ctypes.c_int64 * 2)()
+        _lib.check(self._h, self._L.admp_plane_spread_stats(self._h, out, 1 if reset else 0), 'admp_plane_spread_stats')
+        return {'records': int(out[0]), 'computed': int(out[1])}
+
     def plane_mfma_stats(self, reset=False):
         out = (ctypes.c_int64 * 2)()
         _lib.check(self._h, self._L.admp_plane_mfma_stats(self._h, out, 1 if reset else 0), 'admp_plane_mfma_stats')
diff --git a/include/admp_hip.h b/include/admp_hip.h
--- a/include/admp_hip.h
+++ b/include/admp_hip.h
@@ -186,6 +186,7 @@
 int admp_xpass_stats(admp_handle* h, int64_t* out2, int reset);
 int admp_plane_mfma_stats(admp_handle* h, int64_t* out2, int reset);
 int admp_plane_mfma_stats4(admp_handle* h, int64_t* out4, int reset);
+int admp_plane_spread_stats(admp_handle* h, int64_t* out2, int reset);
 #define ADMP_MESH_INFO_WORDS 16
 #define ADMP_MESH_PATH_ROCFFT 0
 #define ADMP_MESH_PATH_FUSED_X 1
```

Result: no change. 551.4 ns/day (median of 4 runs) (+0.3%).
